# graphic-goose/ferreus_rbf_rs

Measured on AMD Instinct MI355X. Metric: BBFMM matvecs/s, higher is better.
Workload: dtype f64; 1 GPU; 10000000 uniform 3D points, LinearRbf, order 7, 1 rhs, adaptive sparse tree, ACA eps=1e-7, set_weights + evaluate at the sources; points=10000000, kernel=LinearRbf, order=7, nrhs=1, parallelism=single GPU

## Files before the change

ferreus_rbf_rs_amd/_lib.py:

```python
from __future__ import annotations

import ctypes
import os

HERE = os.path.dirname(os.path.abspath(__file__))
LIB_PATH = os.environ.get("FERREUS_BBFMM_HIP_LIB") or os.path.join(HERE, "libferreus_bbfmm_hip.so")

OK, POINT_OUTSIDE_TREE, KERNEL_NO_GRADIENTS, BAD_ARGUMENT, DEVICE_ERROR, UNSUPPORTED = range(6)
FLAG_HOST_ONLY = 1
FLAG_M2L_SHARED_BASIS = 2
FLAG_DIRECT_SMALL_W_LEAVES = 4
FLAG_DETERMINISTIC = 8
N_PHASES = 11
PHASE_NAMES = ["gather", "P2M", "M2M", "M2L_stage1", "M2L_stage2", "P2L", "L2L", "P2P", "M2P",
               "L2P", "scatter"]

c_i32, c_i64, c_f64, c_u32 = ctypes.c_int32, ctypes.c_int64, ctypes.c_double, ctypes.c_uint32
c_p = ctypes.c_void_p


class Params(ctypes.Structure):
    _fields_ = [("max_points_per_cell", c_i64), ("compression_type", c_i32),
                ("epsilon", c_f64), ("eval_chunk_size", c_i64)]

# ... 56 lines not shown
    "bbfmm_isosurface_cluster_tables": (ctypes.c_int, [c_p, c_p, c_p]),
    "bbfmm_isosurface_curvature_tables": (ctypes.c_int, [c_p, c_p, c_p]),
    "bbfmm_isosurface_curvature_weight": (ctypes.c_int, [c_p, c_p, c_i32, c_p, c_p, c_p, c_p]),
    "bbfmm_isosurface_curvature_stats": (ctypes.c_int, [c_p, c_i32, c_p]),
    "bbfmm_isosurface_count": (c_i32, [c_p]),
    "bbfmm_isosurface_size": (ctypes.c_int, [c_p, c_i32, c_p, c_p]),
    "bbfmm_isosurface_copy": (ctypes.c_int, [c_p, c_i32, c_p, c_p]),
    "bbfmm_isosurface_error": (ctypes.c_char_p, [c_p]),
    "bbfmm_isosurface_destroy": (None, [c_p]),
    "bbfmm_prepare_target_subset": (ctypes.c_int, [c_p, c_p, c_i64]),
    "bbfmm_fast_matrix_vector_product": (ctypes.c_int, [c_p, c_p, c_i64, c_i64, c_p, c_i64, c_p,
                                                        c_i64, c_f64, c_p]),
    "bbfmm_matvec_device": (ctypes.c_int, [c_p, c_p, c_i64, c_i32, c_p, c_i64, c_i32]),
    "bbfmm_target_subset_create": (ctypes.c_int, [c_p, c_p, c_i64, c_p]),
    "bbfmm_matvec_subset_device": (ctypes.c_int, [c_p, c_i32, c_p, c_p, c_i32]),
    "bbfmm_stream": (c_p, [c_p]),
    "bbfmm_set_partition": (ctypes.c_int, [c_p, c_i32, c_i32]),
    "bbfmm_partition_row_count": (c_i64, [c_p]),
    "bbfmm_partition_rows": (ctypes.c_int, [c_p, c_p]),
    "bbfmm_partition_coarse_count": (c_i64, [c_p]),
    "bbfmm_matvec_partition_upward": (ctypes.c_int, [c_p, c_p, c_i64, c_i32, c_p, c_p]),
    "bbfmm_matvec_partition_finish": (ctypes.c_int, [c_p, c_p, c_p, c_i64, c_i32, c_p]),
    "bbfmm_partition_world": (c_i32, [c_p]),
    "bbfmm_partition_rank": (c_i32, [c_p]),
    "bbfmm_partition_bounds": (ctypes.c_int, [c_p, c_i32, c_p]),
    "bbfmm_matvec_partition_finish_sorted": (ctypes.c_int, [c_p, c_p, c_p, c_i64, c_p]),
    "bbfmm_partition_scatter": (ctypes.c_int, [c_p, c_p, c_i32, c_i32, c_i64, c_i32, c_p, c_i64]),
    "bbfmm_debug_partition_upward_counts": (ctypes.c_int, [c_p, c_p, c_p, c_p]),
    "bbfmm_debug_host_copy_rates": (ctypes.c_int, [c_i64, c_p]),
    "bbfmm_get_tree_stats": (ctypes.c_int, [c_p, c_p]),
    "bbfmm_tree_built_on_device": (ctypes.c_int, [c_p]),
    "bbfmm_last_evaluate_at_sources": (ctypes.c_int, [c_p]),
    "bbfmm_debug_targets_are_sources": (ctypes.c_int, [c_p, c_p, c_i64, c_i64]),
    "bbfmm_debug_rows_of_sources": (ctypes.c_int, [c_p, c_p, c_i64, c_i64, c_p]),
    "bbfmm_get_cells": (ctypes.c_int, [c_p, c_p, c_p]),
    "bbfmm_get_leaf_sources": (ctypes.c_int, [c_p, c_p, c_p]),
    "bbfmm_get_list": (ctypes.c_int, [c_p, ctypes.c_char, c_p, c_p, c_p]),
    "bbfmm_get_m2l_ranks": (ctypes.c_int, [c_p, c_p, c_p]),
    "bbfmm_get_m2l_operator": (ctypes.c_int, [c_p, c_i32, c_i32, c_p]),
    "bbfmm_get_m2l_factors": (ctypes.c_int, [c_p, c_i32, c_i32, c_p, c_p]),
    "bbfmm_get_permutation_tables": (ctypes.c_int, [c_p, c_p, c_p, c_p, c_p, c_p]),
    "bbfmm_points_to_leaves": (ctypes.c_int, [c_p, c_p, c_i64, c_i64, c_p, c_p]),
    "bbfmm_set_profiling": (ctypes.c_int, [c_p, c_i32]),
    "bbfmm_get_phase_ms": (ctypes.c_int, [c_p, c_p, c_p]),
    "bbfmm_reset_phase_ms": (ctypes.c_int, [c_p]),
    "bbfmm_mfma_f64_selftest": (ctypes.c_int, [c_p, c_p, c_p]),
    "bbfmm_fp64_valu_selftest": (ctypes.c_int, [c_p, c_p]),
    "bbfmm_debug_kernel_values": (ctypes.c_int, [c_i32, c_i32, ctypes.c_double, ctypes.c_double, c_p, c_i64, c_p, c_p, c_p]),
    "bbfmm_debug_math": (ctypes.c_int, [c_i32, c_i32, c_p, c_i64, c_p, c_p]),
    "bbfmm_debug_dense_m2m": (ctypes.c_int, [c_p, c_i32, c_p]),
    "bbfmm_debug_apply_m2l_tables_host": (ctypes.c_int, [c_p, c_p, c_p]),
    "bbfmm_debug_m2l_variants": (ctypes.c_int, [c_p, c_p, c_p]),
    "bbfmm_debug_m2l_pairs": (ctypes.c_int, [c_p, c_p, c_i64, c_p, c_p]),
    "bbfmm_debug_m2l_pairs_stage2": (ctypes.c_int, [c_p, c_p, c_i64, c_p, c_p]),
    "bbfmm_debug_m2l_s2_last_ksplit": (ctypes.c_int, [c_p, c_p]),
    "bbfmm_debug_get_coefficients": (ctypes.c_int, [c_p, ctypes.c_char, c_i32, c_p]),
    "bbfmm_debug_morton_encode": (ctypes.c_uint64, [c_i32, c_p, ctypes.c_uint64]),
    "bbfmm_debug_morton_decode": (None, [c_i32, ctypes.c_uint64, c_p, c_p]),
    "bbfmm_debug_morton_neighbours": (c_i32, [c_i32, ctypes.c_uint64, c_p]),
    "bbfmm_debug_direction_vectors": (c_i32, [c_i32, c_p]),
    "bbfmm_debug_reference_vectors": (ctypes.c_int, [c_p, c_p, c_p]),
    "bbfmm_givens_rotation": (None, [c_f64, c_f64, c_p, c_p, c_p]),
    "bbfmm_fgmres": (ctypes.c_int, [c_i64, c_p, c_p, c_p, c_p, c_p, c_p, c_i32, c_i32, c_i32, c_f64,
                                    c_p, c_p, c_p, c_p, c_p]),
    "bbfmm_schwarz_ddm_solver": (ctypes.c_int, [c_i64, c_p, c_p, c_p, c_p, c_p, c_i32, c_i32, c_f64,
                                                c_p, c_p, c_p, c_p, c_p]),
    "bbfmm_rbf_system_apply": (ctypes.c_int, [c_p, c_p, c_p, c_i64]),
    "bbfmm_ddm_params_defaults": (None, [c_p]),
    "bbfmm_ddm_params_for_points": (None, [c_i64, c_p]),
    "bbfmm_ddm_build": (ctypes.c_int, [c_p, c_i64, c_i32, c_i64, c_p, c_p]),
    "bbfmm_ddm_destroy": (None, [c_p]),
    "bbfmm_ddm_num_levels": (c_i32, [c_p]),
    "bbfmm_ddm_level_size": (c_i64, [c_p, c_i32]),
    "bbfmm_ddm_level_points": (ctypes.c_int, [c_p, c_i32, c_p]),
    "bbfmm_ddm_num_domains": (c_i64, [c_p, c_i32]),
    "bbfmm_ddm_domain_size": (c_i64, [c_p, c_i32, c_i64]),
    "bbfmm_ddm_domain": (ctypes.c_int, [c_p, c_i32, c_i64, c_p, c_p, c_p]),
    "bbfmm_schwarz_create": (ctypes.c_int, [c_p, c_p, c_i64, c_i32, c_i64, c_p, c_p, c_p]),
    "bbfmm_schwarz_create_sharded": (ctypes.c_int, [c_p, c_p, c_i64, c_i32, c_i64, c_p, c_p, c_i32, c_i32, c_p, c_i64, c_p, c_p, c_p]),
    "bbfmm_schwarz_factor_bytes": (c_i64, [c_p]),
    "bbfmm_schwarz_domains_owned": (c_i64, [c_p, c_i32, ctypes.POINTER(c_i64), ctypes.POINTER(c_i64)]),
    "bbfmm_schwarz_destroy": (None, [c_p]),
    "bbfmm_schwarz_basis_size": (c_i64, [c_p]),
    "bbfmm_schwarz_num_levels": (c_i32, [c_p]),
    "bbfmm_schwarz_monomial_matrix": (c_p, [c_p]),
    "bbfmm_debug_evaluate_monomials": (ctypes.c_int, [c_p, c_i64, c_i32, c_i64, c_i32, c_p, c_p, c_p]),
    "bbfmm_schwarz_apply": (ctypes.c_int, [c_p, c_p, c_p, c_i64]),
    "bbfmm_schwarz_level_size": (c_i64, [c_p, c_i32]),
    "bbfmm_schwarz_level_points": (ctypes.c_int, [c_p, c_i32, c_p]),
    "bbfmm_schwarz_debug_level_solve": (ctypes.c_int, [c_p, c_i32, c_p, c_p, c_i64, c_i32]),
    "bbfmm_ddm_debug_level_create": (ctypes.c_int, [c_p, c_i64, c_i32, c_i64, c_i64, c_p, c_p, c_p, c_p, c_i32, c_i32, c_p]),
    "bbfmm_ddm_debug_level_destroy": (None, [c_p]),
    "bbfmm_ddm_debug_level_info": (ctypes.c_int, [c_p, c_p]),
    "bbfmm_ddm_debug_level_layout": (ctypes.c_int, [c_p, c_p, c_p, c_p, c_p, c_p]),
    "bbfmm_ddm_debug_level_assembled": (ctypes.c_int, [c_p, c_p]),
    "bbfmm_ddm_debug_level_factor": (ctypes.c_int, [c_p, c_p]),
    "bbfmm_ddm_debug_level_solve": (ctypes.c_int, [c_p, c_p, c_p, c_i64, c_i32]),
}


class Interpolant(ctypes.Structure):
    _fields_ = [("kernel_type", c_i32), ("polynomial_degree", c_i32), ("nugget", c_f64), ("base_range", c_f64),
                ("total_sill", c_f64), ("flags", c_u32)]


FLAG_GLOBAL_SCALING = 1
# ... 49 lines not shown
```

ferreus_rbf_rs_amd/csrc/capi.cpp:

```cpp
#include <cmath>
#include <cstddef>
#include <cstring>
#include <new>
#include <string>
#include <vector>

#include <algorithm>
#include <chrono>
#include <cstdlib>
#include <memory>

#include "device_group.hpp"
#include "ferreus_bbfmm_hip.h"
#include "fmm_tree.hpp"
#include "isosurface.hpp"
#include "isosurface_curvature.hpp"
#include "isosurface_intersect.hpp"
#include "morton.hpp"

struct bbfmm_handle {
    bbfmm::FmmTree tree;
    std::unique_ptr<bbfmm::DeviceGroup> group;
    std::string err;
};
// ... 1221 lines not shown

int bbfmm_debug_apply_m2l_tables_host(const bbfmm_handle *h, const double *M, double *L) {
    if (!h || !M || !L) return BBFMM_BAD_ARGUMENT;
    return h->tree.debug_apply_m2l_tables_host(M, L);
}

uint64_t bbfmm_debug_morton_encode(int32_t d, const uint64_t *anchor, uint64_t level) {
    if (d < 1 || d > 3 || !anchor) return 0;
    return bbfmm::encode_morton_point(anchor, level, d);
}
void bbfmm_debug_morton_decode(int32_t d, uint64_t key, uint64_t *anchor_out, uint64_t *level_out) {
    if (d < 1 || d > 3 || !anchor_out || !level_out) return;
    bbfmm::decode_key(key, d, anchor_out, level_out);
}
int32_t bbfmm_debug_morton_neighbours(int32_t d, uint64_t key, uint64_t *keys_out) {
    if (d < 1 || d > 3 || !keys_out) return -1;
    return bbfmm::get_neighbours(key, d, keys_out);
}
int32_t bbfmm_debug_direction_vectors(int32_t d, int32_t *out) {
    if (d < 1 || d > 3 || !out) return -1;
    const int(*dirs)[3];
    const int n = bbfmm::direction_vectors(d, &dirs);
    for (int i = 0; i < n; ++i)
        for (int a = 0; a < d; ++a) out[i * d + a] = dirs[i][a];
    return n;
}
int bbfmm_debug_reference_vectors(const bbfmm_handle *h, int32_t *out, int32_t *n_ref_out) {
    if (!h) return BBFMM_BAD_ARGUMENT;
    const bbfmm::Operators &ops = h->tree.ops();
    if (n_ref_out) *n_ref_out = ops.n_ref;
    if (out) std::copy(ops.ref_vecs.begin(), ops.ref_vecs.end(), out);
    return BBFMM_OK;
}

int bbfmm_debug_m2l_variants(const bbfmm_handle *h, int64_t *n_variants, int64_t *n_cells) {
    if (!h) return BBFMM_BAD_ARGUMENT;
    int64_t nv = 0, nc = 0;
    h->tree.m2l_variant_stats(&nv, &nc);
    if (n_variants) *n_variants = nv;
    if (n_cells) *n_cells = nc;
    return BBFMM_OK;
}

int bbfmm_debug_m2l_pairs(const bbfmm_handle *h, int32_t *out, int64_t cap, int64_t *n_out, int32_t *pairs_on) {
    if (!h || !n_out) return BBFMM_BAD_ARGUMENT;
    std::vector<int32_t> v;
    h->tree.debug_m2l_pairs(&v);
    *n_out = static_cast<int64_t>(v.size());
    if (pairs_on) *pairs_on = h->tree.m2l_pairs() ? 1 : 0;
    if (out) std::copy(v.begin(), v.begin() + std::min<int64_t>(cap, *n_out), out);
    return BBFMM_OK;
}

int bbfmm_debug_m2l_pairs_stage2(const bbfmm_handle *h, int32_t *out, int64_t cap, int64_t *n_out, int32_t *pairs_on) {
    if (!h || !n_out) return BBFMM_BAD_ARGUMENT;
    std::vector<int32_t> v;
    h->tree.debug_m2l_pairs_stage2(&v);
    *n_out = static_cast<int64_t>(v.size());
    if (pairs_on) *pairs_on = h->tree.m2l_pairs_stage2() ? 1 : 0;
    if (out) std::copy(v.begin(), v.begin() + std::min<int64_t>(cap, *n_out), out);
    return BBFMM_OK;
}

int bbfmm_debug_m2l_s2_last_ksplit(const bbfmm_handle *h, int32_t *ksplit) {
    if (!h || !ksplit) return BBFMM_BAD_ARGUMENT;
    *ksplit = h->tree.debug_m2l_s2_last_ksplit();
    return BBFMM_OK;
}

int bbfmm_debug_get_coefficients(bbfmm_handle *h, char which, int32_t k, double *out) {
    GUARD(h) return h->tree.debug_get_coefficients(which, k, out);
    END_GUARD(h)
}

}

#include "ddm.hpp"
struct bbfmm_ddm {
    bbfmm::DdmTree tree;
};
extern "C" {
void bbfmm_ddm_params_defaults(bbfmm_ddm_params *out) {
    if (!out) return;
    const bbfmm::DdmParams p;
    out->leaf_threshold = p.leaf_threshold;
    out->overlap_quota = p.overlap_quota;
    out->coarse_ratio = p.coarse_ratio;
    out->coarse_threshold = p.coarse_threshold;
}

void bbfmm_ddm_params_for_points(int64_t n, bbfmm_ddm_params *out) {
    if (!out) return;
    bbfmm_ddm_params_defaults(out);
    out->coarse_threshold = std::max<int64_t>(out->coarse_threshold, n / 470 + 1);
}
int bbfmm_ddm_build(const double *points, int64_t n, int32_t d, int64_t ld, const bbfmm_ddm_params *params,
                    bbfmm_ddm **out) {
    if (!out) return BBFMM_BAD_ARGUMENT;
    *out = nullptr;
    bbfmm::DdmParams p;
    if (params) {
        p.leaf_threshold = params->leaf_threshold;
        p.overlap_quota = params->overlap_quota;
        p.coarse_ratio = params->coarse_ratio;
        p.coarse_threshold = params->coarse_threshold;
    }
// ... 53 lines not shown
```

ferreus_rbf_rs_amd/csrc/device.hpp:

```cpp
#pragma once
#include <hip/hip_runtime.h>

#include <cstdint>

#include "kernels.hpp"

namespace bbfmm {

constexpr int kMaxOrder = 16;
constexpr int kM2lTile = 128;
constexpr int kM2lS1Block = 176;
constexpr int kM2lS1BlockPairs = 160;
constexpr int kM2lSlotWindow = 128;
constexpr int kM2lBlkTwoDst = 1 << 30;

struct DevCheb {
    int p, d, n, n_pad;
    double polyn[kMaxOrder * kMaxOrder];
    double nodes[kMaxOrder];
    double xfer[2 * kMaxOrder * kMaxOrder];
};

struct ChebRef {
    const DevCheb *dev;
    int p, d, n, n_pad;
};

struct M2lClass {
    const double *vt_all;
    const int32_t *row_dst;
    const int32_t *row_dst2;
    const int32_t *blk_t0;
    int32_t n_rows;
    int32_t r_pad16;
    int32_t n_t;
    const double *u_all;
    int32_t k_pad;
    int32_t kp;
    const int32_t *cells;
    int32_t n_cells;
    const int32_t *cslot;
    const int64_t *cbase;
};

struct M2lTileDesc {
    int32_t level_class;
    int32_t first;
    int32_t count;
    int32_t q_first;
    int32_t q_count;
    int32_t pad;
};

void launch_gather_weights(const double *w, int64_t ldw, int K, const int32_t *order, int64_t N,
                           double *w_sorted, hipStream_t s);
void launch_gather_weights_subset(const double *w, int64_t ldw, int K, const int32_t *order, const int32_t *pos, int64_t n_pos,
                                  int64_t N, double *w_sorted, hipStream_t s);
constexpr int kMaxScatterParts = 64;
struct ScatterParts {
    int n;
    int64_t bound[kMaxScatterParts + 1];
};
void launch_scatter_parts(const double *all, const ScatterParts &parts, int64_t m_max, int K, const int32_t *order, double *out,
                          int64_t ldo, hipStream_t s);
void launch_sum_slots(const double *slots, int n_slots, int64_t len, double *out, hipStream_t s);
void launch_scatter_output(const double *out_sorted, int64_t n, int K, const int32_t *perm,
                           double *out, int64_t ldo, int accumulate, hipStream_t s);
void launch_gather_rows(const double *src, int64_t ld_src, int ncols, const int32_t *idx, int64_t n,
                        double *dst, int64_t ld_dst, hipStream_t s);

void launch_p2m(const ChebRef &ch, const double *const *src_xyz, const double *w_sorted, int64_t N,
                int K, int64_t C, const int32_t *leaf_cells, int n_leaves, const int32_t *pt_begin,
                const int32_t *pt_end, const double *centers, const double *lengths, double *M,
                hipStream_t s);
int launch_m2m(const ChebRef &ch, int K, int64_t C, const int32_t *parents, int n_parents,
               const int64_t *child_ptr, const int32_t *child_idx, const int32_t *octant, double *M,
               hipStream_t s);
int launch_l2l(const ChebRef &ch, int K, int64_t C, const int32_t *cells, int n_cells,
               const int32_t *parent, const int32_t *octant, const uint8_t *active, double *L,
               hipStream_t s);

void launch_m2l_stage1(const M2lClass *classes, const M2lTileDesc *tiles, const int32_t *tile_idx, int n_tiles,
                       int n_pad, int max_slot_t, int K, int64_t C, const double *M, double *cbuf,
                       int64_t cbuf_len, hipStream_t s, bool own_blocks = false, int max_blocks = 8, int ne16 = 0);
void launch_m2l_parity(const double *M, int n_pad, double *Mp, int n_par, int ne16, int n_e, int n_o, int p, int64_t rows,
                       hipStream_t s);
void launch_m2l_stage2(const M2lClass *classes, const M2lTileDesc *tiles, const int32_t *tile_idx, int n_tiles,
                       int n_pad, int K, int64_t C, const double *cbuf, int64_t cbuf_len,
                       const uint16_t *qlist, double *L, hipStream_t s, bool allow_ksplit = true);
struct M2lS2PairsPlan {
    int ga, gb, ce, co;
    int ne16() const { return 16 * ga * ce; }
    int n_par() const { return 16 * (ga * ce + gb * co); }
};
M2lS2PairsPlan m2l_s2_pairs_plan(int groups_even, int groups_odd);
bool launch_m2l_stage2_pairs(const M2lClass *classes, const M2lTileDesc *tiles, const int32_t *tile_idx, int n_tiles,
                             const M2lS2PairsPlan &plan, int K, int64_t C, const double *cbuf, int64_t cbuf_len,
                             const uint16_t *qlist, double *Lp, hipStream_t s, bool allow_ksplit = true, int *ksplit_out = nullptr);
void launch_m2l_unparity(const double *Lp, int n_par, int ne16, double *L, int n, int n_pad, int n_e, int n_o, int p, int64_t rows,
                         hipStream_t s);
void launch_m2l_zero_segments(const int32_t *segs, int64_t n_segs, int K, double *cbuf, int64_t cbuf_len, hipStream_t s);
void launch_m2l_basis(const M2lClass *classes, const M2lTileDesc *tiles, int n_tiles, int in_ld, int out_ld, int K,
                      int64_t C, const double *in, double *out, hipStream_t s);
void launch_small_gemm(bool trans_a, int M, int N, int Kd, const double *A, int64_t lda, const double *B, int64_t ldb,
                       double *Cm, int64_t ldc, hipStream_t s);

struct M2lAssembleTv {
    int32_t perm;
    int32_t rank;
    int32_t row;
    int64_t vt_off;
    int64_t u_off;
};
struct M2lAssembleClass {
    const M2lAssembleTv *src, *tgt;
    int32_t n_src, n_tgt, r_pad16, k_pad, max_rank;
    int32_t n_e, n_o, ne16, n_par, p;
    int32_t u_npar, u_ne16, u_rows, u_ne, u_no;
};
void launch_m2l_assemble(const M2lAssembleClass &c, int n, int n_pad, bool compressed, const double *ops,
                         const int32_t *invperm, double *vt_all, double *u_all, hipStream_t s);

struct DirectJobs {
    int n_jobs;
    const int32_t *job_cell;
    const int32_t *tgt_begin, *tgt_end;
    const int64_t *run_ptr;
    const int32_t *runs;
};
void launch_p2p(const KernelSpec &ks, int d, const DirectJobs &jobs, const double *const *tgt_xyz,
                int64_t n_tgt, const double *const *src_xyz, const double *w_sorted, int64_t N, int K,
                double *out_sorted, double *grad_sorted, hipStream_t s);
constexpr int kSymMaxRhs = 4;
void launch_p2p_sym(const KernelSpec &ks, int n_jobs, const int32_t *tgt_begin, const int32_t *tgt_end,
                    const int64_t *run_range, int n_leaf_jobs, const int32_t *l_tgt_begin, const int32_t *l_tgt_end,
                    const int64_t *l_run_range, int n_wave_jobs, const int32_t *w_tgt_begin, const int32_t *w_tgt_end,
                    const int64_t *w_run_range, const int32_t *runs3, int32_t tgt_off, const double *const *src_xyz,
                    const double *w_sorted, int64_t ldw, int K, double *out_sorted, int64_t ldo, hipStream_t s);
int p2p_sym_rows_per_job();
int p2p_sym3_rows_per_job();
int p2p_sym_wave_rows();
int64_t p2p_sym_wave_min_jobs();
int wx_sym_rows_per_job();
int wx_sym3_rows_per_job();
void launch_wx_sym(const KernelSpec &ks, const ChebRef &ch, int n_jobs, const int32_t *tgt_begin, const int32_t *tgt_end,
                   const int64_t *w_range, int n_leaf_jobs, const int32_t *l_tgt_begin, const int32_t *l_tgt_end,
                   const int64_t *l_w_range, const int32_t *w_cells, const double *centers, const double *lengths,
                   const double *const *src_xyz, const double *w_sorted, int64_t ldw, int K, const double *M, double *L,
                   int64_t ld_ml, double *out_sorted, int64_t ldo, int out_off, int out_n, hipStream_t s);
void launch_m2p(const KernelSpec &ks, const ChebRef &ch, int n_jobs, const int32_t *tgt_begin,
                const int32_t *tgt_end, const int64_t *w_begin, const int64_t *w_end,
                const int32_t *w_cells,
                const double *centers, const double *lengths, const double *const *tgt_xyz,
                int64_t n_tgt, int K, int64_t C, const double *M, double *out_sorted,
                double *grad_sorted, hipStream_t s);
void launch_p2l(const KernelSpec &ks, const ChebRef &ch, int n_jobs, const int32_t *cells,
                const int64_t *run_ptr, const int32_t *runs, const double *centers,
                const double *lengths, const double *const *src_xyz, const double *w_sorted,
                int64_t N, int K, int64_t C, double *L, hipStream_t s);
void launch_l2p(const ChebRef &ch, int n_jobs, const int32_t *leaf_cells, const int32_t *tgt_begin,
                const int32_t *tgt_end, const double *centers, const double *lengths,
                const double *const *tgt_xyz, int64_t n_tgt, int K, int64_t C, const double *L,
                double *out_sorted, double *grad_sorted, hipStream_t s);

bool l2p_order_supported(int p, int d);

int mfma_f64_selftest(double *tflops, int *layout_errors, double *info);
int valu_f64_selftest(double *tflops, double *mhz);
int debug_kernel_values_device(const KernelSpec &ks, const double *r2, int64_t n, double *value, double *value_g, double *factor);
int debug_math_device(int which, const double *x, int64_t n, double *out, double *out2);

// ... 2 lines not shown
```

ferreus_rbf_rs_amd/csrc/device_m2l.hip:

```cpp
#include "device_common.hpp"

#include <cmath>

namespace bbfmm {

typedef __attribute__((address_space(3))) void *lptr_t;

__device__ inline unsigned lds_offset(const double *p) {
    return static_cast<unsigned>(reinterpret_cast<uintptr_t>((lptr_t)p));
}
__device__ inline unsigned uniform_u32(unsigned v) { return __builtin_amdgcn_readfirstlane(v); }
__device__ inline const double *uniform_ptr(const double *p) {
    const uintptr_t v = reinterpret_cast<uintptr_t>(p);
    const unsigned lo = __builtin_amdgcn_readfirstlane(static_cast<unsigned>(v));
    const unsigned hi = __builtin_amdgcn_readfirstlane(static_cast<unsigned>(v >> 32));
    return reinterpret_cast<const double *>((static_cast<uintptr_t>(hi) << 32) | lo);
}
__device__ inline void dma16(const double *g, unsigned lds_wave_byte_offset) {
    asm volatile("s_mov_b32 m0, %1\n\ts_nop 0\n\tglobal_load_lds_dwordx4 %0, off" ::"v"(g),
                 "s"(uniform_u32(lds_wave_byte_offset))
                 : "memory");
}
__device__ inline void dma4(const int32_t *g, unsigned lds_wave_byte_offset) {
    asm volatile("s_mov_b32 m0, %1\n\ts_nop 0\n\tglobal_load_lds_dword %0, off" ::"v"(g),
                 "s"(uniform_u32(lds_wave_byte_offset))
                 : "memory");
}
__device__ inline void wait_dma_and_barrier() {
    asm volatile("s_waitcnt vmcnt(0)" ::: "memory");
    __syncthreads();
}
template <int N> __device__ inline void wait_dma_keep_stores_and_barrier() {
    asm volatile("s_waitcnt vmcnt(%0)" ::"n"(N < 63 ? N : 63) : "memory");
    __syncthreads();
}
template <int N> __device__ inline double add_row_ror(double v) {
    const int lo = __double2loint(v), hi = __double2hiint(v);
    const int rlo = __builtin_amdgcn_update_dpp(0, lo, 0x120 + N, 0xf, 0xf, false);
    const int rhi = __builtin_amdgcn_update_dpp(0, hi, 0x120 + N, 0xf, 0xf, false);
    return v + __hiloint2double(rhi, rlo);
}

__device__ inline void dma16s(const double *sbase, unsigned voff_bytes, unsigned lds_wave_byte_offset) {
    asm volatile("s_mov_b32 m0, %2\n\ts_nop 0\n\tglobal_load_lds_dwordx4 %0, %1" ::"v"(voff_bytes),
                 "s"(uniform_ptr(sbase)), "s"(uniform_u32(lds_wave_byte_offset))
                 : "memory");
}

template <int NG16, int STAGE, int MINW, bool PAIRS = false>
__global__ __launch_bounds__(512, MINW) void m2l_gemm_k4(const M2lClass *__restrict__ classes,
                                                  const M2lTileDesc *__restrict__ tiles, int n_pad, int g16_0,
                                                  int64_t C, const double *__restrict__ in, int64_t in_len,
                                                  double *__restrict__ out, int64_t out_len,
                                                  const uint16_t *__restrict__ qlist, int slot_t,
                                                  const int32_t *__restrict__ tile_idx) {
    extern __shared__ double lds[];
    const M2lTileDesc tile = tiles[blockIdx.x];
    const M2lClass cls = classes[tile.level_class];
    const int kr = blockIdx.y;
    const int tid = threadIdx.x, wave = tid >> 6, lane = tid & 63;
    constexpr int BLK = PAIRS ? kM2lS1BlockPairs : kM2lS1Block;
    const int n_zb = STAGE == 1 ? cls.r_pad16 / BLK : 1;
    const bool own_blocks = STAGE == 1 && tile.pad == 2;
    const int zb0 = STAGE == 1 ? (own_blocks ? tile.q_first : (int)((int64_t)n_zb * blockIdx.z / gridDim.z)) : 0;
    const int zb1 = STAGE == 1 ? (own_blocks ? tile.q_first + tile.q_count : (int)((int64_t)n_zb * (blockIdx.z + 1) / gridDim.z)) : 1;
    const int ld = STAGE == 1 ? cls.r_pad16 : n_pad;
    const int ksplit = STAGE == 2 && slot_t > 1 ? slot_t : 1;
    const int zcols = STAGE == 2 ? (int)gridDim.z / ksplit : 1;
    const int zk = STAGE == 2 ? (int)blockIdx.z / zcols : 0, zc = STAGE == 2 ? (int)blockIdx.z - zk * zcols : (int)blockIdx.z;
    const int q_lo = STAGE == 2 ? tile.q_count * zk / ksplit : 0;
    const int nq = STAGE == 1 ? n_pad / 16 : STAGE == 2 ? tile.q_count * (zk + 1) / ksplit - q_lo : (int)(in_len / 16);
    const uint16_t *ql = qlist + tile.q_first + q_lo;
    const int nq_e = PAIRS ? (int)(in_len / 16) : 0;
    if (zb0 >= zb1) return;
    const int g16 = g16_0 + (STAGE >= 2 ? zc * NG16 : 0);
    const double *opbase = (STAGE == 1 ? cls.vt_all : cls.u_all) + 16 * g16;

    constexpr int OP_CHUNKS = 2 * NG16;
    constexpr int NCH = (OP_CHUNKS + 7) / 8;
    constexpr int OP_DOUBLES = OP_CHUNKS * 128;
    constexpr int BUF = OP_DOUBLES + 2048;

    constexpr int NP = NG16 / 2, NS = NG16 & 1;
    unsigned voff[NCH];
#pragma unroll
    for (int i = 0; i < NCH; ++i) {
        const int c = wave + 8 * i;
        if (c < 4 * NP) {
            const int e = c / NP, pr = c - e * NP, k = lane >> 4, p = lane & 15;
            voff[i] = (unsigned)(((4 * k + e) * ld + 32 * pr + 2 * p) * 8);
        } else {
            const int e = 2 * (c - 4 * NP) + (lane >> 5), r = lane & 31, k = r >> 3, pair = r & 7;
            voff[i] = (unsigned)(((4 * k + e) * ld + 32 * NP + 2 * pair) * 8);
        }
    }
    auto cell_p = [&](int pos) {
        const int q = pos < tile.count ? pos : 0;
        return tile.pad ? tile_idx[tile.first + q] : tile.first + q;
    };
    const double *cptr[2];
#pragma unroll
    for (int h = 0; h < 2; ++h) {
        const int tg = 2 * h + (lane >> 5), eh = (lane >> 4) & 1, k = (lane >> 2) & 3, j = lane & 3;
        const int pos = wave * 16 + 4 * tg + j;
        const int p = cell_p(pos);
        const int64_t base = STAGE == 2 ? (int64_t)kr * in_len + cls.cbase[p]
                                        : ((int64_t)kr * C + cls.cells[p]) * (STAGE == 1 ? (int64_t)n_pad : in_len);
        cptr[h] = in + base + 4 * k + 2 * eh;
    }
    const unsigned lds0 = lds_offset(lds);
    const int64_t qstride = (int64_t)16 * ld;
    auto stage = [&](int sidx, int buf) {
        const int zb = zb0 + sidx / nq, qi = sidx - (sidx / nq) * nq;
        const int q = STAGE == 2 ? (int)ql[qi] : qi;
#pragma unroll
        for (int i = 0; i < NCH; ++i)
            if (wave + 8 * i < OP_CHUNKS)
                dma16s(opbase + (int64_t)zb * BLK + q * qstride, voff[i],
                       lds0 + (unsigned)(buf * BUF + (wave + 8 * i) * 128) * 8u);
#pragma unroll
        for (int h = 0; h < 2; ++h)
            dma16(cptr[h] + 16 * q, lds0 + (unsigned)(buf * BUF + OP_DOUBLES + (2 * wave + h) * 128) * 8u);
    };

    double acc[4][NG16];
    double acc_e[4][PAIRS ? NG16 : 1];
#pragma unroll
    for (int tg = 0; tg < 4; ++tg)
#pragma unroll
        for (int g = 0; g < NG16; ++g) {
            acc[tg][g] = 0.0;
            if constexpr (PAIRS) acc_e[tg][g] = 0.0;
        }

    const int bk = lane >> 4, bj = lane & 3;
    const bool wave_live = wave * 16 < tile.count;
    const int n_steps = (zb1 - zb0) * nq;
    const int di = lane >> 4, db = (lane >> 2) & 3, dj = lane & 3;
    constexpr int AUX = PAIRS ? 384 : 192;
    const int32_t *aux = reinterpret_cast<const int32_t *>(lds + 2 * BUF);
    int32_t *ptab = reinterpret_cast<int32_t *>(lds + 2 * BUF) + 2 * AUX;
    const int32_t *slds = aux + 2 * AUX + 128 + wave * 16 * slot_t;
    if (STAGE == 1 && lane < 16) ptab[wave * 16 + lane] = cell_p(wave * 16 + lane);
    const unsigned aux0 = lds0 + (unsigned)(2 * BUF) * 8u;
    auto stage_cols = [&](int zb_, int par) {
        if (STAGE == 1 && 64 * wave <= 16 * NG16) {
            const int e = 64 * wave + lane;
            const int32_t *src = e < 16 * NG16 ? cls.row_dst + zb_ * BLK + 16 * g16 + e : cls.blk_t0 + zb_;
            dma4(src, aux0 + (unsigned)(par * AUX + 64 * wave) * 4u);
        } else if (PAIRS && 64 * wave < 192 + 16 * NG16) {
            const int e = 64 * wave + lane - 192;
            const int32_t *src = e < 16 * NG16 ? cls.row_dst2 + zb_ * BLK + 16 * g16 + e : cls.blk_t0 + zb_;
            dma4(src, aux0 + (unsigned)(par * AUX + 64 * wave) * 4u);
        }
    };
    const int slot_sh = 31 - __builtin_clz(slot_t | 1);
    auto stage_slots = [&](int par) {
        const int t0 = __builtin_amdgcn_readfirstlane(aux[par * AUX + 16 * NG16]) & (kM2lBlkTwoDst - 1);
        const unsigned dst0 = aux0 + (unsigned)(2 * AUX + 128 + wave * 16 * slot_t) * 4u;
        for (int i = 0; i < slot_t / 4; ++i) {
            const int e = i * 64 + lane, cl = e >> slot_sh, tl = e & (slot_t - 1);
            const int32_t *src = cls.cslot + (int64_t)ptab[wave * 16 + cl] * cls.n_t + min(t0 + tl, cls.n_t - 1);
            dma4(src, dst0 + (unsigned)i * 256u);
        }
    };
    if (n_steps > 0) {
        stage(0, 0);
// ... 184 lines not shown
                                int n_pad, int n_colblocks, int K, int64_t C, const double *in, int64_t in_len,
                                double *out, int64_t out_len, const uint16_t *qlist, int slot_t,
                                const int32_t *tile_idx, hipStream_t s) {
    int done = 0;
    const int pref = m2l_chunk_pref<STAGE>();
    while (done < total_groups) {
        const int left = total_groups - done;
        int take;
#define M2L_GO(NG, MW)                                                                                              \
    {                                                                                                               \
        take = NG;                                                                                                  \
        m2l_gemm_launch<NG, STAGE, MW>(classes, tiles, n_tiles, n_pad, done,                                        \
                                       STAGE >= 2 ? 1 : n_colblocks, K, C, in, in_len,                            \
                                       out, out_len, qlist, slot_t, tile_idx, s);                                   \
    }
        if (STAGE >= 2 && !(n_colblocks == 1 && left >= 16)) {
            int best_ng = 2, best_z = 1;
            for (int ng : {11, 8, 7, 6, 4, 2})
                for (int zc = 1; zc <= (n_colblocks == 1 ? 1 : ng == 11 ? 2 : 3); ++zc)
                    if (ng * zc <= left && ((left - ng * zc) % 2 == 0 || left - ng * zc == 7) &&
                        (ng * zc > best_ng * best_z || (ng * zc == best_ng * best_z && ng > best_ng))) {
                        best_ng = ng;
                        best_z = zc;
                    }
            take = best_ng * best_z;
#define M2L_ZGO(NG, MW)                                                                                             \
    m2l_gemm_launch<NG, STAGE, MW>(classes, tiles, n_tiles, n_pad, done, best_z, K, C, in, in_len, out, out_len,    \
                                   qlist, slot_t, tile_idx, s);
            if constexpr (STAGE >= 2) {
                switch (best_ng) {
                case 11: M2L_ZGO(11, 1) break;
                case 8: M2L_ZGO(8, 4) break;
                case 7: M2L_ZGO(7, 2) break;
                case 6: M2L_ZGO(6, 4) break;
                case 4: M2L_ZGO(4, 4) break;
                default: M2L_ZGO(2, 4) break;
                }
            }
#undef M2L_ZGO
        } else if (pref == 22 && left >= 22) M2L_GO(22, 1)
        else if (pref == 22 && left >= 16) M2L_GO(16, 1)
        else if (pref == 11 && left >= 11) M2L_GO(11, 1)
        else if (left >= 8) M2L_GO(8, 4)
        else if (left >= 6) M2L_GO(6, 4)
        else if (left >= 4) M2L_GO(4, 4)
        else M2L_GO(2, 4)
#undef M2L_GO
        done += take;
    }
}

void launch_m2l_stage1(const M2lClass *classes, const M2lTileDesc *tiles, const int32_t *tile_idx, int n_tiles,
                       int n_pad, int max_slot_t, int K, int64_t C, const double *M, double *cbuf, int64_t cbuf_len,
                       hipStream_t s, bool own_blocks, int max_blocks, int ne16) {
    if (n_tiles == 0) return;
    int slot_t = 16;
    while (slot_t < max_slot_t) slot_t *= 2;
    const int n_cu = device_cu_count();
    const int zmax = n_tiles * 8 < n_cu ? std::max(8, std::min(max_blocks, 32)) : 8;
    int zsplit = 1;
    double best = 1e300;
    for (int z = 1; z <= zmax; ++z) {
        const double rounds = std::ceil(static_cast<double>(n_tiles) * z / n_cu);
        const double cost = rounds / z * (1.0 + 0.005 * z);
        if (cost < best - 1e-12) {
            best = cost;
            zsplit = z;
        }
    }
    const int n_colblocks = own_blocks ? 1 : zsplit;
    if (ne16 > 0) {
        m2l_gemm_launch<kM2lS1BlockPairs / 16, 1, 1, true>(classes, tiles, n_tiles, n_pad, 0, n_colblocks, K, C, M, ne16, cbuf, cbuf_len,
                                                      nullptr, slot_t, tile_idx, s);
        return;
    }
    m2l_dispatch_chunks<1>(kM2lS1Block / 16, classes, tiles, n_tiles, n_pad, n_colblocks, K, C, M, 0, cbuf, cbuf_len, nullptr,
                           slot_t, tile_idx, s);
}

static int m2l_s2_ksplit(int64_t wgs, bool allow_ksplit) {
    static const int ks_env = [] {
        const int v = env_int("BBFMM_M2L_S2_KSPLIT", 0);
        return v >= 1 && v <= 32 ? v : 0;
    }();
    if (!allow_ksplit) return 1;
    if (ks_env > 0) return ks_env;
    const int n_cu = device_cu_count();
    int ksplit = 1;
    if (wgs * 2 <= static_cast<int64_t>(kM2lS2KsplitFill) * n_cu) {
        double best = 1e300;
        for (int ks = 1; ks <= 16; ++ks) {
            const double cost = std::ceil(static_cast<double>(wgs * ks) / n_cu) * (0.05 + 1.0 / ks);
            if (cost < best - 1e-12) {
                best = cost;
                ksplit = ks;
            }
        }
    }
    return ksplit;
}

void launch_m2l_stage2(const M2lClass *classes, const M2lTileDesc *tiles, const int32_t *tile_idx, int n_tiles,
                       int n_pad, int K, int64_t C, const double *cbuf, int64_t cbuf_len, const uint16_t *qlist,
                       double *L, hipStream_t s, bool allow_ksplit) {
    if (n_tiles == 0) return;
    static const int z = env_int("BBFMM_M2L_S2_ZSPLIT", 2) == 1 ? 1 : 2;
    const int ksplit = m2l_s2_ksplit(static_cast<int64_t>(n_tiles) * z * K, allow_ksplit);
    m2l_dispatch_chunks<2>(n_pad / 16, classes, tiles, n_tiles, n_pad, z, K, C, cbuf, cbuf_len, L, 0, qlist, ksplit > 1 ? ksplit : 0, tile_idx, s);
}

template <int NG16>
__device__ __forceinline__ void m2l_s2_pairs_body(const M2lClass &cls, const M2lTileDesc &tile, int n_par, int g16, bool odd,
                                                  int zk, int ksplit, int64_t C, const double *__restrict__ in, int64_t in_len,
                                                  double *__restrict__ out, const uint16_t *__restrict__ qlist,
                                                  const int32_t *__restrict__ tile_idx, double *lds) {
    const int kr = blockIdx.y;
    const int tid = threadIdx.x, wave = tid >> 6, lane = tid & 63;
    const int ld = n_par;
    const int q_lo = tile.q_count * zk / ksplit;
    const int nq = tile.q_count * (zk + 1) / ksplit - q_lo;
    const uint16_t *ql = qlist + tile.q_first + q_lo;
    const int kp = cls.kp, kp16 = kp >> 4;
    const double *opbase = cls.u_all + 16 * g16;

    constexpr int OP_CHUNKS = 2 * NG16;
// ... 189 lines not shown
}

__global__ __launch_bounds__(256) void m2l_unparity_kernel(const double *__restrict__ Lp, int n_par, int ne16, double *__restrict__ L,
                                                           int n, int n_pad, int n_e, int n_o, int p, int p1, int64_t rows) {
    const int64_t row = static_cast<int64_t>(blockIdx.x) * 4 + (threadIdx.x >> 6);
    if (row >= rows) return;
    const double *src = Lp + row * n_par;
    double *dst = L + row * n_pad;
    for (int j = threadIdx.x & 63; j < n_e; j += 64) {
        const double e = src[j];
        if (j < n_o) {
            const double o = src[ne16 + j];
            dst[j] = e + o;
            dst[j + (p - 1 - 2 * (j / p1)) * p1] = e - o;
        } else {
            dst[j] = e;
        }
    }
    for (int j = n + (threadIdx.x & 63); j < n_pad; j += 64) dst[j] = 0.0;
}

void launch_m2l_unparity(const double *Lp, int n_par, int ne16, double *L, int n, int n_pad, int n_e, int n_o, int p, int64_t rows,
                         hipStream_t s) {
    if (rows <= 0) return;
    const int p1 = n_e / ((p + 1) / 2);
    hipLaunchKernelGGL(m2l_unparity_kernel, dim3(static_cast<unsigned>((rows + 3) / 4)), dim3(256), 0, s, Lp, n_par, ne16, L, n, n_pad, n_e,
                       n_o, p, p1, rows);
}

__global__ __launch_bounds__(256) void m2l_parity_kernel(const double *__restrict__ M, int n_pad, double *__restrict__ Mp, int n_par,
                                                         int ne16, int n_e, int n_o, int p, int p1, int64_t rows) {
    const int64_t row = static_cast<int64_t>(blockIdx.x) * 4 + (threadIdx.x >> 6);
    if (row >= rows) return;
    const double *src = M + row * n_pad;
    double *dst = Mp + row * n_par;
    for (int j = threadIdx.x & 63; j < n_e; j += 64) {
        const double v = src[j];
        if (j < n_o) {
            const double w = src[j + (p - 1 - 2 * (j / p1)) * p1];
            dst[j] = v + w;
            dst[ne16 + j] = v - w;
        } else {
            dst[j] = v;
        }
    }
}

void launch_m2l_parity(const double *M, int n_pad, double *Mp, int n_par, int ne16, int n_e, int n_o, int p, int64_t rows,
                       hipStream_t s) {
    if (rows <= 0) return;
    const int p1 = n_e / ((p + 1) / 2);
    hipLaunchKernelGGL(m2l_parity_kernel, dim3(static_cast<unsigned>((rows + 3) / 4)), dim3(256), 0, s, M, n_pad, Mp, n_par, ne16, n_e,
                       n_o, p, p1, rows);
}

__global__ __launch_bounds__(256) void m2l_zero_segments_kernel(const int32_t *__restrict__ segs, int64_t n_segs,
                                                                double *__restrict__ cbuf, int64_t cbuf_len) {
    const int64_t sg = (static_cast<int64_t>(blockIdx.x) * 256 + threadIdx.x) >> 4;
    const int l = threadIdx.x & 15;
    if (sg >= n_segs) return;
    const int2 e = reinterpret_cast<const int2 *>(segs)[sg];
    double2 *dst = reinterpret_cast<double2 *>(cbuf + static_cast<int64_t>(blockIdx.y) * cbuf_len) + e.x;
    for (int i = l; i < e.y; i += 16) dst[i] = make_double2(0.0, 0.0);
}

void launch_m2l_zero_segments(const int32_t *segs, int64_t n_segs, int K, double *cbuf, int64_t cbuf_len, hipStream_t s) {
    if (n_segs <= 0) return;
    hipLaunchKernelGGL(m2l_zero_segments_kernel, dim3(static_cast<unsigned>((n_segs * 16 + 255) / 256), K), dim3(256), 0, s, segs,
                       n_segs, cbuf, cbuf_len);
}

void launch_m2l_basis(const M2lClass *classes, const M2lTileDesc *tiles, int n_tiles, int in_ld, int out_ld, int K,
                      int64_t C, const double *in, double *out, hipStream_t s) {
    if (n_tiles == 0) return;
    m2l_dispatch_chunks<3>(out_ld / 16, classes, tiles, n_tiles, out_ld, 2, K, C, in, in_ld, out, 0, nullptr, 0, nullptr, s);
}

template <bool TA>
__global__ __launch_bounds__(256) void small_gemm_kernel(int M, int N, int Kd, const double *__restrict__ A, int64_t lda,
                                                         const double *__restrict__ B, int64_t ldb, double *__restrict__ Cm,
                                                         int64_t ldc) {
    __shared__ double sa[16][64 + 1], sb[16][64 + 1];
    const int tx = threadIdx.x & 15, ty = threadIdx.x >> 4;
    const int i0 = blockIdx.y * 64, j0 = blockIdx.x * 64;
    double acc[4][4] = {};
    for (int k0 = 0; k0 < Kd; k0 += 16) {
        for (int e = threadIdx.x; e < 16 * 64; e += 256) {
            const int kk = TA ? e >> 6 : e & 15, ii = TA ? e & 63 : e >> 4;
            const int k = k0 + kk, i = i0 + ii;
            sa[kk][ii] = (k < Kd && i < M) ? (TA ? A[(int64_t)k * lda + i] : A[(int64_t)i * lda + k]) : 0.0;
        }
        for (int e = threadIdx.x; e < 16 * 64; e += 256) {
            const int kk = e >> 6, jj = e & 63;
            const int k = k0 + kk, j = j0 + jj;
            sb[kk][jj] = (k < Kd && j < N) ? B[(int64_t)k * ldb + j] : 0.0;
        }
        __syncthreads();
#pragma unroll
        for (int kk = 0; kk < 16; ++kk) {
            double a[4], b[4];
#pragma unroll
            for (int r = 0; r < 4; ++r) a[r] = sa[kk][ty + 16 * r];
#pragma unroll
            for (int c = 0; c < 4; ++c) b[c] = sb[kk][tx + 16 * c];
#pragma unroll
            for (int r = 0; r < 4; ++r)
// ... 9 lines not shown
            const int i = i0 + ty + 16 * r, j = j0 + tx + 16 * c;
            if (i < M && j < N) Cm[(int64_t)i * ldc + j] = acc[r][c];
        }
}

void launch_small_gemm(bool trans_a, int M, int N, int Kd, const double *A, int64_t lda, const double *B, int64_t ldb,
                       double *Cm, int64_t ldc, hipStream_t s) {
    if (M <= 0 || N <= 0) return;
    const dim3 grid((N + 63) / 64, (M + 63) / 64);
    if (trans_a) hipLaunchKernelGGL(small_gemm_kernel<true>, grid, dim3(256), 0, s, M, N, Kd, A, lda, B, ldb, Cm, ldc);
    else hipLaunchKernelGGL(small_gemm_kernel<false>, grid, dim3(256), 0, s, M, N, Kd, A, lda, B, ldb, Cm, ldc);
}

__global__ __launch_bounds__(256) void assemble_vt_kernel(M2lAssembleClass c, int n, int n_pad, int compressed,
                                                          const double *__restrict__ ops, const int32_t *__restrict__ invperm,
                                                          double *__restrict__ vt_all) {
    const int64_t t = static_cast<int64_t>(blockIdx.x) * 256 + threadIdx.x;
    if (t >= static_cast<int64_t>(c.n_src) * n) return;
    const int pos = static_cast<int>(t / n), m = static_cast<int>(t % n);
    const M2lAssembleTv tv = c.src[pos];
    const int im = invperm[static_cast<int64_t>(tv.perm) * n + m];
    double *dst = vt_all + static_cast<int64_t>(m) * c.r_pad16 + tv.row;
    if (compressed) {
        const double *src = ops + tv.vt_off + static_cast<int64_t>(im) * tv.rank;
        for (int kk = 0; kk < tv.rank; ++kk) dst[kk] = src[kk];
    } else {
        dst[im] = 1.0;
    }
}

__global__ __launch_bounds__(256) void assemble_vt_parity_kernel(M2lAssembleClass c, int n, const double *__restrict__ ops,
                                                                 const int32_t *__restrict__ invperm, double *__restrict__ vt_all) {
    const int64_t t = static_cast<int64_t>(blockIdx.x) * 256 + threadIdx.x;
    if (t >= static_cast<int64_t>(c.n_src) * c.n_e) return;
    const int pos = static_cast<int>(t / c.n_e), j = static_cast<int>(t % c.n_e);
    const M2lAssembleTv tv = c.src[pos];
    const int p1 = n / c.p;
    const int rj = j + (c.p - 1 - 2 * (j / p1)) * p1;
    const int32_t *inv = invperm + static_cast<int64_t>(tv.perm) * n;
    const double *s0 = ops + tv.vt_off + static_cast<int64_t>(inv[j]) * tv.rank;
    const double *s1 = ops + tv.vt_off + static_cast<int64_t>(inv[rj]) * tv.rank;
    double *de = vt_all + static_cast<int64_t>(j) * c.r_pad16 + tv.row;
    double *dod = vt_all + static_cast<int64_t>(c.ne16 + j) * c.r_pad16 + tv.row;
    if (j >= c.n_o) {
        for (int kk = 0; kk < tv.rank; ++kk) de[kk] = s0[kk];
    } else {
        for (int kk = 0; kk < tv.rank; ++kk) {
            de[kk] = 0.5 * (s0[kk] + s1[kk]);
            dod[kk] = 0.5 * (s0[kk] - s1[kk]);
        }
    }
}

__global__ __launch_bounds__(256) void assemble_u_kernel(M2lAssembleClass c, int n, int n_pad, const double *__restrict__ ops,
                                                         const int32_t *__restrict__ invperm, double *__restrict__ u_all) {
    const int pos = blockIdx.y;
    const M2lAssembleTv tv = c.tgt[pos];
    const int64_t t = static_cast<int64_t>(blockIdx.x) * 256 + threadIdx.x;
    if (t >= static_cast<int64_t>(tv.rank) * n) return;
    const int kk = static_cast<int>(t / n), i = static_cast<int>(t % n);
    u_all[static_cast<int64_t>(tv.row + kk) * n_pad + i] = ops[tv.u_off + static_cast<int64_t>(kk) * n + invperm[static_cast<int64_t>(tv.perm) * n + i]];
}

__global__ __launch_bounds__(256) void assemble_u_parity_kernel(M2lAssembleClass c, int n, const double *__restrict__ ops,
                                                                const int32_t *__restrict__ invperm, double *__restrict__ u_all) {
    const M2lAssembleTv tv = c.tgt[blockIdx.y];
    const int64_t t = static_cast<int64_t>(blockIdx.x) * 256 + threadIdx.x;
    if (t >= static_cast<int64_t>(tv.rank) * c.u_ne) return;
    const int kk = static_cast<int>(t / c.u_ne), i = static_cast<int>(t % c.u_ne);
    const int p1 = n / c.p;
    const int ri = i + (c.p - 1 - 2 * (i / p1)) * p1;
    const int32_t *inv = invperm + static_cast<int64_t>(tv.perm) * n;
    const double *ucol = ops + tv.u_off + static_cast<int64_t>(kk) * n;
    double *dst = u_all + static_cast<int64_t>(tv.row + kk) * c.u_npar;
    const double a = ucol[inv[i]];
    if (i >= c.u_no) {
        dst[i] = a;
    } else {
        const double b = ucol[inv[ri]];
        dst[i] = 0.5 * (a + b);
        dst[c.u_ne16 + i] = 0.5 * (a - b);
    }
}

void launch_m2l_assemble(const M2lAssembleClass &c, int n, int n_pad, bool compressed, const double *ops,
                         const int32_t *invperm, double *vt_all, double *u_all, hipStream_t s) {
    (void)hipMemsetAsync(vt_all, 0, static_cast<size_t>(c.n_e > 0 ? c.n_par : n_pad) * c.r_pad16 * sizeof(double), s);
    (void)hipMemsetAsync(u_all, 0, (c.u_npar > 0 ? static_cast<size_t>(c.u_rows) * c.u_npar : static_cast<size_t>(c.k_pad) * n_pad) * sizeof(double), s);
    if (c.n_src > 0 && c.n_e > 0)
        hipLaunchKernelGGL(assemble_vt_parity_kernel, dim3(static_cast<unsigned>((static_cast<int64_t>(c.n_src) * c.n_e + 255) / 256)), dim3(256),
                           0, s, c, n, ops, invperm, vt_all);
    else if (c.n_src > 0)
        hipLaunchKernelGGL(assemble_vt_kernel, dim3(static_cast<unsigned>((static_cast<int64_t>(c.n_src) * n + 255) / 256)), dim3(256), 0, s, c, n, n_pad,
                           compressed ? 1 : 0, ops, invperm, vt_all);
    if (c.n_tgt > 0 && c.max_rank > 0 && c.u_npar > 0)
        hipLaunchKernelGGL(assemble_u_parity_kernel, dim3(static_cast<unsigned>((static_cast<int64_t>(c.max_rank) * c.u_ne + 255) / 256), c.n_tgt),
                           dim3(256), 0, s, c, n, ops, invperm, u_all);
    else if (c.n_tgt > 0 && c.max_rank > 0)
        hipLaunchKernelGGL(assemble_u_kernel, dim3(static_cast<unsigned>((static_cast<int64_t>(c.max_rank) * n + 255) / 256), c.n_tgt), dim3(256), 0, s, c,
                           n, n_pad, ops, invperm, u_all);
}

}
```

ferreus_rbf_rs_amd/csrc/fmm_m2l_tables.cpp:

```cpp
#include "fmm_tree_impl.hpp"

namespace bbfmm {

void FmmTree::fill_m2l_operator_arrays(const HostM2lClass &hc, std::vector<double> *vt_all,
                                       std::vector<double> *u_all) const {
    const int n_pad = round_up(ops_.n, 32);
    vt_all->resize(static_cast<size_t>(m2l_pairs_ ? m2l_npar_ : n_pad) * hc.r_pad16);
    u_all->resize(m2l_pairs2_ ? static_cast<size_t>(hc.k_pad - hc.kp) * m2l_s2_plan_.n_par() : static_cast<size_t>(hc.k_pad) * n_pad);
    fill_m2l_operator_arrays(hc, vt_all->data(), u_all->data());
}

void FmmTree::fill_m2l_operator_arrays(const HostM2lClass &hc, double *vt_all, double *u_all) const {
    const int n = ops_.n, n_pad = round_up(n, 32);
    const bool compressed = ops_.compression != kCompressionNone;
    const auto &lops = ops_.m2l[hc.level];
    auto zero = [](double *p, size_t len) {
        parallel_for_chunks(static_cast<int64_t>(len), int64_t(1) << 18, [&](int64_t b, int64_t e) {
            std::memset(p + b, 0, static_cast<size_t>(e - b) * sizeof(double));
        });
    };
    zero(vt_all, static_cast<size_t>(m2l_pairs_ ? m2l_npar_ : n_pad) * hc.r_pad16);
    zero(u_all, m2l_pairs2_ ? static_cast<size_t>(hc.k_pad - hc.kp) * m2l_s2_plan_.n_par() : static_cast<size_t>(hc.k_pad) * n_pad);
    struct RowSrc {
        const M2lOperator *op;
        const int32_t *inv;
        int first_row;
    };
    std::vector<RowSrc> row_src;
    for (size_t pos = 0; pos < hc.src_tv.size(); ++pos) {
        if (m2l_pairs_ && hc.src_pair[pos] == -2) continue;
        const int tv = hc.src_tv[pos];
        const M2lOperator &op = lops[ops_.ref_lookup[tv]];
        row_src.push_back(RowSrc{&op, &ops_.invperm[static_cast<size_t>(ops_.perm_lookup[tv]) * n], hc.src_row0[pos]});
    }
    if (m2l_pairs_) {
        parallel_for(m2l_ne_, 8, [&](int64_t j) {
            const bool centre = j >= m2l_no_;
            const int rj = m2l_rho(static_cast<int>(j));
            double *de = vt_all + static_cast<size_t>(j) * hc.r_pad16;
            double *dod = vt_all + static_cast<size_t>(m2l_ne16_ + j) * hc.r_pad16;
            for (const RowSrc &rs : row_src) {
                const int r = rs.op->rank;
                const double *s0 = &rs.op->vt[static_cast<size_t>(rs.inv[j]) * r], *s1 = &rs.op->vt[static_cast<size_t>(rs.inv[rj]) * r];
                for (int kk = 0; kk < r; ++kk) {
                    if (centre) {
                        de[rs.first_row + kk] = s0[kk];
                    } else {
                        de[rs.first_row + kk] = 0.5 * (s0[kk] + s1[kk]);
                        dod[rs.first_row + kk] = 0.5 * (s0[kk] - s1[kk]);
                    }
                }
            }
        });
    } else {
        parallel_for(n, 8, [&](int64_t m) {
            double *dst = vt_all + static_cast<size_t>(m) * hc.r_pad16;
            for (const RowSrc &rs : row_src) {
                const int r = rs.op->rank;
                const int im = rs.inv[m];
                if (compressed) {
                    const double *src = &rs.op->vt[static_cast<size_t>(im) * r];
                    for (int kk = 0; kk < r; ++kk) dst[rs.first_row + kk] = src[kk];
                } else {
                    dst[rs.first_row + im] = 1.0;
                }
            }
        });
    }
    if (m2l_pairs2_) {
        const int n_par = m2l_s2_plan_.n_par(), ne16 = m2l_s2_plan_.ne16();
        parallel_for(static_cast<int64_t>(hc.tgt_tv.size()), 1, [&](int64_t pos) {
            if (hc.tgt_pair[pos] == -2) return;
            const int tv = hc.tgt_tv[pos];
            const M2lOperator &op = lops[ops_.ref_lookup[tv]];
            const int32_t *inv = &ops_.invperm[static_cast<size_t>(ops_.perm_lookup[tv]) * n];
            const int row0 = hc.tgt_off[pos] - (hc.tgt_pair[pos] >= 0 ? 0 : hc.kp);
            for (int kk = 0; kk < op.rank; ++kk) {
                double *dst = u_all + static_cast<size_t>(row0 + kk) * n_par;
                const double *ucol = &op.u[static_cast<size_t>(kk) * n];
                for (int i = 0; i < m2l_ne_; ++i) {
                    const double a = ucol[inv[i]], b = ucol[inv[m2l_rho(i)]];
                    if (i >= m2l_no_) {
                        dst[i] = a;
                    } else {
                        dst[i] = 0.5 * (a + b);
                        dst[ne16 + i] = 0.5 * (a - b);
                    }
                }
// ... 22 lines not shown
    m2l_variants_.clear();
    m2l_tiles1_h_.clear();
    m2l_tile_idx1_h_.clear();
    m2l_classes_h_.clear();
    m2l_tiles_h_.clear();
    m2l_qlist_h_.clear();
    m2l_batches_.clear();
    m2l_batch_of_class_.clear();
    m2l_group_ops_.clear();
    cbuf_batch_len_ = 0;
    cbuf_total_len_ = 0;
    m2l_flops_k1_ = 0;
    m2l_flops_level_.clear();
    if (t.depth < 2) return BBFMM_OK;
    if (!host_only_) {
        size_t free_b = 0, total_b = 0;
        if (hipMemGetInfo(&free_b, &total_b) == hipSuccess && total_b > 0)
            m2l_budget_bytes_ = std::max<int64_t>(int64_t(4) << 30, static_cast<int64_t>(total_b / 16));
    }
    if (const char *e = std::getenv("BBFMM_M2L_CBUF_MB")) {
        const double mb = std::atof(e);
        if (mb > 0) m2l_budget_bytes_ = static_cast<int64_t>(mb * 1048576.0);
    }

    auto comp = [&](int tv, int a) { return ops_.all_vecs[static_cast<size_t>(tv) * d + a]; };
    {
        const char *e = std::getenv("BBFMM_M2L_S1_PAIRS");
        m2l_pairs_ = !(e && std::atoi(e) == 0) && compressed && !shared_basis_ && d >= 2 && ops_.p >= 2;
        const char *e2 = std::getenv("BBFMM_M2L_S2_PAIRS");
        m2l_pairs2_ = !(e2 && std::atoi(e2) == 0) && compressed && !shared_basis_ && d >= 2 && ops_.p >= 2;
        m2l_partner_.assign(static_cast<size_t>(nvec), -1);
        m2l_s1_block_ = m2l_pairs_ ? kM2lS1BlockPairs : kM2lS1Block;
        const int p1 = n / ops_.p;
        m2l_ne_ = (ops_.p + 1) / 2 * p1;
        m2l_no_ = ops_.p / 2 * p1;
        m2l_ne16_ = round_up(m2l_ne_, 16);
        m2l_npar_ = m2l_ne16_ + round_up(m2l_no_, 16);
        m2l_s2_plan_ = m2l_s2_pairs_plan(m2l_ne16_ / 16, round_up(m2l_no_, 16) / 16);
        for (int tv = 0; tv < nvec && (m2l_pairs_ || m2l_pairs2_); ++tv) {
            if (comp(tv, 0) == 0) continue;
            int rt = -1;
            for (int u = 0; u < nvec && rt < 0; ++u) {
                bool same = comp(u, 0) == -comp(tv, 0);
                for (int a = 1; a < d; ++a) same = same && comp(u, a) == comp(tv, a);
                if (same) rt = u;
            }
            if (rt < 0 || ops_.ref_lookup[rt] != ops_.ref_lookup[tv]) continue;
            const int32_t *it = &ops_.invperm[static_cast<size_t>(ops_.perm_lookup[tv]) * n];
            const int32_t *ir = &ops_.invperm[static_cast<size_t>(ops_.perm_lookup[rt]) * n];
            bool ok = true;
            for (int m = 0; m < n && ok; ++m) ok = ir[m] == it[m2l_rho(m)];
            if (ok) m2l_partner_[static_cast<size_t>(tv)] = rt;
        }
    }
    auto far = [&](int tv) {
        int mx = 0;
        for (int a = 0; a < d; ++a) mx = std::max(mx, std::abs(comp(tv, a)));
        return mx >= 2;
    };
    std::vector<std::vector<int>> tgt_list(ncls), src_list(ncls), tpos_tgt(ncls, std::vector<int>(nvec, -1)),
        tpos_src(ncls, std::vector<int>(nvec, -1));
    for (int o = 0; o < ncls; ++o)
        for (int tv = 0; tv < nvec; ++tv) {
            if (!far(tv)) continue;
            bool okt = true, oks = true;
            for (int a = 0; a < d; ++a) {
                const int oa = (o >> a) & 1, ta = comp(tv, a);
                okt = okt && ta >= oa - 3 && ta <= oa + 2;
                oks = oks && ta >= -2 - oa && ta <= 3 - oa;
            }
            if (okt) {
                tpos_tgt[o][tv] = static_cast<int>(tgt_list[o].size());
                tgt_list[o].push_back(tv);
            }
            if (oks) {
                tpos_src[o][tv] = static_cast<int>(src_list[o].size());
                src_list[o].push_back(tv);
            }
        }
    auto pairs_first = [&](std::vector<int> *list, std::vector<int> *tpos) {
        std::vector<int> ordered, singles;
        std::vector<uint8_t> used(static_cast<size_t>(nvec), 0);
        for (int tv : *list) {
            const int rt = m2l_partner_[static_cast<size_t>(tv)];
            if (used[static_cast<size_t>(tv)]) continue;
            if (rt >= 0 && (*tpos)[rt] >= 0 && m2l_partner_[static_cast<size_t>(rt)] == tv) {
                const int first = comp(tv, 0) > 0 ? tv : rt;
                ordered.push_back(first);
                ordered.push_back(first == tv ? rt : tv);
                used[static_cast<size_t>(tv)] = used[static_cast<size_t>(rt)] = 1;
            } else {
                singles.push_back(tv);
            }
        }
        ordered.insert(ordered.end(), singles.begin(), singles.end());
        *list = ordered;
        for (size_t i = 0; i < ordered.size(); ++i) (*tpos)[ordered[i]] = static_cast<int>(i);
    };
    for (int o = 0; o < ncls; ++o) {
        if (m2l_pairs_) pairs_first(&src_list[o], &tpos_src[o]);
        if (m2l_pairs2_) pairs_first(&tgt_list[o], &tpos_tgt[o]);
    }
    std::vector<std::vector<int32_t>> tgt_pair(ncls);
    for (int o = 0; o < ncls; ++o) {
        const std::vector<int> &tl = tgt_list[o];
        tgt_pair[o].assign(tl.size(), -1);
        for (size_t pos = 0; m2l_pairs2_ && pos + 1 < tl.size(); ++pos)
            if (m2l_partner_[static_cast<size_t>(tl[pos])] == tl[pos + 1] && m2l_partner_[static_cast<size_t>(tl[pos + 1])] == tl[pos]) {
                tgt_pair[o][pos] = static_cast<int32_t>(pos + 1);
                tgt_pair[o][pos + 1] = -2;
                ++pos;
            }
    }
    auto target_class = [&](int o, int tv) {
        int oc = 0;
        for (int a = 0; a < d; ++a) {
            const int v = ((o >> a) & 1) + comp(tv, a);
            oc |= (((v % 2) + 2) % 2) << a;
        }
        return oc;
    };

    std::vector<int32_t> pos_in_class(t.n_cells(), -1);
    int64_t bad_pairs = 0;
    auto slot_layout = [&](int level, std::vector<std::vector<int>> *off_tgt, std::vector<int> *k_pad, std::vector<int> *kp_out = nullptr) {
        const auto &lops = ops_.m2l[level];
        off_tgt->assign(ncls, {});
        k_pad->assign(ncls, 0);
        if (kp_out) kp_out->assign(ncls, 0);
        for (int o = 0; o < ncls; ++o) {
            int lead = 0;
            for (size_t pos = 0; pos < tgt_list[o].size(); ++pos)
                if (tgt_pair[o][pos] >= 0) lead += round_up(lops[ops_.ref_lookup[tgt_list[o][pos]]].rank, 2);
            const int kp = round_up(lead, 16);
            int off = 0, off_s = 2 * kp;
            for (size_t pos = 0; pos < tgt_list[o].size(); ++pos) {
                const int seg = round_up(lops[ops_.ref_lookup[tgt_list[o][pos]]].rank, 2);
                if (tgt_pair[o][pos] >= 0) {
                    (*off_tgt)[o].push_back(off);
                } else if (tgt_pair[o][pos] == -2) {
                    (*off_tgt)[o].push_back(kp + off);
                    off += seg;
                } else {
                    (*off_tgt)[o].push_back(off_s);
                    off_s += seg;
                }
            }
            (*k_pad)[o] = round_up(std::max(off_s, 16), 16);
            if (kp_out) (*kp_out)[o] = kp;
        }
    };
    std::vector<int> level_groups(static_cast<size_t>(t.depth) + 1, 1);
    std::vector<std::vector<int>> batch_of(static_cast<size_t>(t.depth) + 1, std::vector<int>(ncls, -1));
    {
// ... 8 lines not shown
        int64_t cur_len = 0;
        for (int level = 2; level <= t.depth; ++level) {
            int64_t len = 0;
            for (int64_t v : class_len[level]) len += v;
            cbuf_total_len_ += len;
            int G = 1;
            if (len > budget)
                for (G = 2; G < ncls; G *= 2) {
                    int64_t worst = 0;
                    for (int g = 0; g < G; ++g) {
                        int64_t gl = 0;
                        for (int o = g * ncls / G; o < (g + 1) * ncls / G; ++o) gl += class_len[level][o];
                        worst = std::max(worst, gl);
                    }
                    if (worst <= budget) break;
                }
            if (G >= ncls) {
                G = ncls;
                int64_t worst = 0;
                for (int64_t v : class_len[level]) worst = std::max(worst, v);
                if (worst > budget && std::getenv("BBFMM_VERBOSE"))
                    std::fprintf(stderr, "[bbfmm] warning: level %d needs %.1f MB of M2L intermediate per right-hand side even "
                                         "with one batch per target class; the budget of %.1f MB (BBFMM_M2L_CBUF_MB) is exceeded\n",
                                 level, worst * 8.0 / 1048576.0, m2l_budget_bytes_ / 1048576.0);
            }
            level_groups[level] = G;
            if (G == 1 && !m2l_batches_.empty() && m2l_batches_.back().groups == 1 && cur_len + len <= budget) {
                m2l_batches_.back().level_hi = level;
                cur_len += len;
                for (int o = 0; o < ncls; ++o) batch_of[level][o] = static_cast<int>(m2l_batches_.size()) - 1;
                continue;
            }
            for (int g = 0; g < G; ++g) {
                M2lBatch b;
                b.level_lo = b.level_hi = level;
                b.groups = G;
                b.group = g;
                for (int o = g * ncls / G; o < (g + 1) * ncls / G; ++o) batch_of[level][o] = static_cast<int>(m2l_batches_.size());
                m2l_batches_.push_back(b);
            }
            cur_len = len;
        }
    }
    std::vector<std::vector<M2lTileDesc>> tiles1_of_batch(m2l_batches_.size());
    std::vector<int32_t> variant_batch;
    std::vector<std::vector<int32_t>> zero_of_batch(m2l_batches_.size());
    for (int level = 2; level <= t.depth; ++level) {
        const auto &lops = ops_.m2l[level];
        auto rank_of = [&](int tv) { return lops[ops_.ref_lookup[tv]].rank; };
        std::vector<std::vector<int>> off_tgt;
        std::vector<int> k_pad, kp_cls;
        slot_layout(level, &off_tgt, &k_pad, &kp_cls);
        const size_t first_class = m2l_host_.size();
        auto mark_pairs = [&](const std::vector<int> &tvs, std::vector<int32_t> *src_pair, std::vector<int32_t> *row0 = nullptr) {
            src_pair->assign(tvs.size(), -1);
            for (size_t pos = 0; m2l_pairs_ && pos + 1 < tvs.size(); ++pos)
                if (m2l_partner_[static_cast<size_t>(tvs[pos])] == tvs[pos + 1] && m2l_partner_[static_cast<size_t>(tvs[pos + 1])] == tvs[pos]) {
                    (*src_pair)[pos] = static_cast<int32_t>(pos + 1);
                    (*src_pair)[pos + 1] = -2;
                    ++pos;
                }
            if (row0) row0->assign(tvs.size(), 0);
            int rows = 0, blk = -1, blk_first = 0;
            for (size_t pos = 0; pos < tvs.size(); ++pos) {
                if ((*src_pair)[pos] == -2) continue;
                const int r = rank_of(tvs[pos]);
                if (r == 0) continue;
                const int last = (*src_pair)[pos] >= 0 ? static_cast<int>(pos) + 1 : static_cast<int>(pos);
                if (rows / m2l_s1_block_ == blk && last - blk_first + 1 > kM2lSlotWindow) rows = round_up(rows, m2l_s1_block_);
                if (row0) (*row0)[pos] = rows;
                const int b1 = (rows + r - 1) / m2l_s1_block_;
                if (rows / m2l_s1_block_ != blk || b1 != blk) {
                    blk = b1;
                    blk_first = static_cast<int>(pos);
                }
                rows = round_up(rows + r, 2);
            }
            return rows;
        };
        auto stage1_rows = [&](int o, const std::vector<int> &tvs, HostM2lClass *hcp) {
            HostM2lClass &hc = *hcp;
            hc.n_t = static_cast<int>(tvs.size());
            std::vector<int32_t> first_row;
            hc.n_rows = mark_pairs(tvs, &hc.src_pair, &first_row);
            hc.r_pad16 = round_up(std::max(hc.n_rows, 1), m2l_s1_block_);
            hc.row_tpos.assign(hc.r_pad16, -1);
            hc.row_off.assign(hc.r_pad16, 0);
            hc.row_tpos2.assign(hc.r_pad16, -1);
            hc.row_off2.assign(hc.r_pad16, 0);
            hc.src_tv = tvs;
            int row = 0;
            hc.src_row0.assign(tvs.size(), 0);
            hc.src_row1.assign(tvs.size(), 0);
            for (size_t pos = 0; pos < tvs.size(); ++pos) {
                if (hc.src_pair[pos] == -2) {
                    hc.src_row0[pos] = hc.src_row0[pos - 1];
                    hc.src_row1[pos] = hc.src_row1[pos - 1];
                    continue;
                }
                const int tv = tvs[pos];
                const int oc = target_class(o, tv);
                const int base_off = off_tgt[oc][tpos_tgt[oc][tv]];
                int base_off2 = 0;
                if (hc.src_pair[pos] >= 0) {
                    const int tv2 = tvs[pos + 1], oc2 = target_class(o, tv2);
                    base_off2 = off_tgt[oc2][tpos_tgt[oc2][tv2]];
                }
                if (rank_of(tv) > 0) row = first_row[pos];
                hc.src_row0[pos] = row;
                for (int kk = 0; kk < rank_of(tv); ++kk, ++row) {
                    hc.row_tpos[row] = static_cast<int32_t>(pos);
                    hc.row_off[row] = base_off + kk;
                    if (hc.src_pair[pos] >= 0) {
                        hc.row_tpos2[row] = static_cast<int32_t>(pos + 1);
                        hc.row_off2[row] = base_off2 + kk;
                    }
                }
                hc.src_row1[pos] = row;
                row = round_up(row, 2);
            }
            const int n_blk = hc.r_pad16 / m2l_s1_block_;
            m2l_max_blocks_ = std::max(m2l_max_blocks_, n_blk);
            hc.blk_t0.assign(n_blk, 0);
            hc.row_dst.assign(hc.r_pad16, -1);
            hc.row_dst2.assign(hc.r_pad16, -1);
            for (int b = 0; b < n_blk; ++b) {
                int t0 = -1, t1 = -1;
                bool two = false;
                for (int r = b * m2l_s1_block_; r < (b + 1) * m2l_s1_block_; ++r) {
                    if (hc.row_tpos[r] < 0) continue;
                    if (t0 < 0) t0 = hc.row_tpos[r];
                    t1 = std::max(hc.row_tpos[r], hc.row_tpos2[r]);
                    two = two || hc.row_tpos2[r] >= 0;
                }
                if (t0 < 0) continue;
                hc.blk_t0[b] = t0 | (two ? kM2lBlkTwoDst : 0);
                m2l_slot_t_ = std::max(m2l_slot_t_, t1 - t0 + 1);
                for (int r = b * m2l_s1_block_; r < (b + 1) * m2l_s1_block_; ++r) {
// ... 120 lines not shown
            const int64_t n_tiles_cls = (static_cast<int64_t>(hc.cells.size()) + kM2lTile - 1) / kM2lTile;
            std::vector<std::vector<uint16_t>> tile_q(static_cast<size_t>(n_tiles_cls));
            parallel_for(n_tiles_cls, 4, [&](int64_t ti) {
                const int32_t first = static_cast<int32_t>(ti * kM2lTile);
                const int32_t count = std::min<int32_t>(kM2lTile, static_cast<int32_t>(hc.cells.size()) - first);
                std::vector<uint8_t> act(static_cast<size_t>(nq), 0);
                for (int32_t i = 0; i < count; ++i) {
                    const int64_t B = hc.cells[first + i];
                    for (int64_t q = t.v.ptr[B]; q < t.v.ptr[B + 1]; ++q) {
                        const int tv = t.v_tidx[q];
                        const int pos = tpos_tgt[o][tv];
                        if (pos < 0) continue;
                        const int a = off_tgt[o][pos] - (off_tgt[o][pos] >= hc.kp ? hc.kp : 0), b = a + rank_of(tv);
                        for (int sq = a / 16; sq <= (b - 1) / 16; ++sq) act[sq] = 1;
                    }
                }
                for (int sq = 0; sq < nq; ++sq)
                    if (act[sq]) tile_q[static_cast<size_t>(ti)].push_back(static_cast<uint16_t>(sq));
            });
            for (int64_t ti = 0; ti < n_tiles_cls; ++ti) {
                M2lTileDesc td;
                td.level_class = static_cast<int32_t>(first_class + o);
                td.first = static_cast<int32_t>(ti * kM2lTile);
                td.count = std::min<int32_t>(kM2lTile, static_cast<int32_t>(hc.cells.size()) - td.first);
                td.pad = 0;
                td.q_first = static_cast<int32_t>(m2l_qlist_h_.size());
                m2l_qlist_h_.insert(m2l_qlist_h_.end(), tile_q[static_cast<size_t>(ti)].begin(), tile_q[static_cast<size_t>(ti)].end());
                td.q_count = static_cast<int32_t>(m2l_qlist_h_.size()) - td.q_first;
                m2l_tiles_h_.push_back(td);
            }
        }
        const int variant_min_tiles = [] {
            const char *e = std::getenv("BBFMM_M2L_VARIANTS");
            return e ? std::atoi(e) : 4;
        }();
        const int G = level_groups[level];
        const bool variants_on = variant_min_tiles > 0 && G == 1;
        for (int g = 0; g < G && G > 1; ++g) {
            const int o_lo = g * ncls / G, o_hi = (g + 1) * ncls / G;
            for (int o = 0; o < ncls; ++o) {
                const HostM2lClass &hc = m2l_host_[first_class + o];
                const size_t nc = hc.cells.size();
                if (nc == 0) continue;
                const int nt = hc.n_t;
                std::vector<int> tvs, keep;
                for (int ps = 0; ps < nt; ++ps) {
                    const int oc = target_class(o, hc.src_tv[ps]);
                    if (oc >= o_lo && oc < o_hi) {
                        tvs.push_back(hc.src_tv[ps]);
                        keep.push_back(ps);
                    }
                }
                if (tvs.empty()) continue;
                HostM2lClass v;
                v.level = level;
                v.octant = o;
                v.k_pad = 16;
                if (!stage1_rows(o, tvs, &v)) return fail(BBFMM_BAD_ARGUMENT, "M2L slot too long for the packed row table");
                v.cells = hc.cells;
                v.cslot.resize(nc * tvs.size());
                {
                    int32_t *dst = v.cslot.data();
                    const int32_t *src = hc.cslot.data();
                    const size_t nk = keep.size();
                    parallel_for_chunks(static_cast<int64_t>(nc), 4096, [&](int64_t lo, int64_t hi) {
                        for (int64_t k = lo; k < hi; ++k)
                            for (size_t q = 0; q < nk; ++q) dst[static_cast<size_t>(k) * nk + q] = src[static_cast<size_t>(k) * nt + keep[q]];
                    });
                }
                const int bidx = batch_of[level][o_lo];
                for (size_t f = 0; f < nc; f += kM2lTile) {
                    M2lTileDesc td;
                    std::memset(&td, 0, sizeof td);
                    td.level_class = -1 - static_cast<int32_t>(m2l_variants_.size());
                    td.first = static_cast<int32_t>(f);
                    td.count = static_cast<int32_t>(std::min<size_t>(kM2lTile, nc - f));
                    td.pad = 0;
                    tiles1_of_batch[static_cast<size_t>(bidx)].push_back(td);
                }
                if (host_only_) fill_m2l_operator_arrays(v, &v.vt_all, &v.u_all);
                m2l_group_ops_[first_class + o].push_back(static_cast<int32_t>(m2l_variants_.size()));
                variant_batch.push_back(bidx);
                m2l_variants_.push_back(std::move(v));
            }
        }
        for (int o = 0; o < ncls && G == 1; ++o) {
            const HostM2lClass &hc = m2l_host_[first_class + o];
            const size_t nc = hc.cells.size();
            if (nc == 0) continue;
            const int nt = hc.n_t;
            std::vector<M2lTileDesc> &tiles1_out = tiles1_of_batch[static_cast<size_t>(batch_of[level][o])];
            std::vector<uint64_t> sig(nc);
            parallel_for(static_cast<int64_t>(nc), 256, [&](int64_t i) {
                uint64_t h = 1469598103934665603ull;
                const int32_t *row = &hc.cslot[static_cast<size_t>(i) * nt];
                uint64_t word = 0;
                for (int ps = 0; ps < nt; ++ps) {
                    word = (word << 1) | (row[ps] >= 0 ? 1u : 0u);
                    if ((ps & 63) == 63 || ps == nt - 1) {
                        h = (h ^ word) * 1099511628211ull;
                        word = 0;
                    }
                }
                sig[static_cast<size_t>(i)] = h;
            });
            auto same_pattern = [&](size_t a, size_t b) {
                if (sig[a] != sig[b]) return false;
                const int32_t *ra = &hc.cslot[a * nt], *rb = &hc.cslot[b * nt];
                for (int ps = 0; ps < nt; ++ps)
                    if ((ra[ps] >= 0) != (rb[ps] >= 0)) return false;
                return true;
            };
            std::vector<int32_t> rest;
            size_t i = 0;
            while (i < nc) {
                size_t j = i + 1;
                while (j < nc && same_pattern(i, j)) ++j;
                size_t full = 0;
                if (variants_on && j - i >= static_cast<size_t>(variant_min_tiles) * kM2lTile) {
                    std::vector<int> tvs;
                    for (int ps = 0; ps < nt; ++ps)
                        if (hc.cslot[i * nt + ps] >= 0) tvs.push_back(hc.src_tv[ps]);
                    std::vector<int32_t> marks;
                    const int present_rows = mark_pairs(tvs, &marks);
                    auto n_pairs = [](const std::vector<int32_t> &m) { return std::count_if(m.begin(), m.end(), [](int32_t v) { return v >= 0; }); };
                    if (!tvs.empty() && (round_up(present_rows, m2l_s1_block_) < hc.r_pad16 || n_pairs(marks) < n_pairs(hc.src_pair))) {
                        full = (j - i) / kM2lTile * kM2lTile;
                        HostM2lClass v;
                        v.level = level;
                        v.octant = o;
                        v.k_pad = 16;
                        if (!stage1_rows(o, tvs, &v)) return fail(BBFMM_BAD_ARGUMENT, "M2L slot too long for the packed row table");
                        v.cells.assign(hc.cells.begin() + static_cast<std::ptrdiff_t>(i), hc.cells.begin() + static_cast<std::ptrdiff_t>(i + full));
                        v.cslot.resize(full * tvs.size());
                        size_t pv = 0;
                        std::vector<int> keep;
                        for (int ps = 0; ps < nt; ++ps)
                            if (hc.cslot[i * nt + ps] >= 0) keep.push_back(ps);
                        for (size_t k = 0; k < full; ++k)
                            for (int ps : keep) v.cslot[pv++] = hc.cslot[(i + k) * nt + ps];
                        for (size_t f = 0; f < full; f += kM2lTile) {
                            M2lTileDesc td;
                            std::memset(&td, 0, sizeof td);
                            td.level_class = -1 - static_cast<int32_t>(m2l_variants_.size());
                            td.first = static_cast<int32_t>(f);
                            td.count = kM2lTile;
                            td.pad = 0;
                            tiles1_out.push_back(td);
                        }
                        if (host_only_) fill_m2l_operator_arrays(v, &v.vt_all, &v.u_all);
                        variant_batch.push_back(batch_of[level][o]);
                        m2l_variants_.push_back(std::move(v));
                    }
                }
                for (size_t k = i + full; k < j; ++k) rest.push_back(static_cast<int32_t>(k));
                i = j;
            }
            for (size_t f = 0; f < rest.size(); f += kM2lTile) {
                M2lTileDesc td;
                std::memset(&td, 0, sizeof td);
                td.level_class = static_cast<int32_t>(first_class + o);
                td.first = static_cast<int32_t>(m2l_tile_idx1_h_.size() + f);
                td.count = static_cast<int32_t>(std::min<size_t>(kM2lTile, rest.size() - f));
                td.pad = 1;
                tiles1_out.push_back(td);
            }
            m2l_tile_idx1_h_.insert(m2l_tile_idx1_h_.end(), rest.begin(), rest.end());
        }
    }
    if (bad_pairs > 0)
        return fail(BBFMM_UNSUPPORTED,
                    "V-list pairs outside the admissible transfer-vector set (source points outside the root box?)");
    m2l_batch_of_class_.assign(m2l_host_.size() + m2l_variants_.size(), 0);
    for (size_t lc = 0; lc < m2l_host_.size(); ++lc)
        m2l_batch_of_class_[lc] = batch_of[static_cast<size_t>(m2l_host_[lc].level)][static_cast<size_t>(m2l_host_[lc].octant)];
    for (size_t v = 0; v < m2l_variants_.size(); ++v) m2l_batch_of_class_[m2l_host_.size() + v] = variant_batch[v];
    m2l_tiles2_h_.clear();
    {
        size_t next = 0;
        for (size_t b = 0; b < m2l_batches_.size(); ++b) {
            M2lBatch &mb = m2l_batches_[b];
            mb.t1_first = static_cast<int32_t>(m2l_tiles1_h_.size());
            for (M2lTileDesc td : tiles1_of_batch[b]) {
                if (td.level_class < 0) td.level_class = static_cast<int32_t>(m2l_host_.size()) + (-1 - td.level_class);
                m2l_tiles1_h_.push_back(td);
            }
            mb.t1_count = static_cast<int32_t>(m2l_tiles1_h_.size()) - mb.t1_first;
            std::vector<M2lTileDesc> part;
            while (next < m2l_tiles_h_.size() && m2l_batch_of_class_[static_cast<size_t>(m2l_tiles_h_[next].level_class)] == static_cast<int32_t>(b))
                part.push_back(m2l_tiles_h_[next++]);
            split_tile_tail(&part, n_cu_);
// ... 228 lines not shown
    const int64_t C = tree_.n_cells();
    double flops = 0.0;
    for (size_t lv = 2; lv < n_levels; ++lv) {
        std::memset(&classes[2 * lv], 0, 2 * sizeof(M2lClass));
        if (basis_rank_[lv] == 0 || lv >= level_cells_.size() || level_cells_[lv].empty()) continue;
        const int rank = basis_rank_[lv];
        std::vector<double> wc(static_cast<size_t>(n_pad) * basis_pad_, 0.0), we(static_cast<size_t>(basis_pad_) * n_pad, 0.0);
        for (int j = 0; j < rank; ++j) {
            const double *col = &basis[lv][static_cast<size_t>(j) * n];
            for (int m = 0; m < n; ++m) {
                wc[static_cast<size_t>(m) * basis_pad_ + j] = col[m];
                we[static_cast<size_t>(j) * n_pad + m] = col[m];
            }
        }
        CHK(dupload(&d_basis_c_[lv], wc));
        CHK(dupload(&d_basis_e_[lv], we));
        const int32_t nc = static_cast<int32_t>(level_cells_[lv].size());
        for (int e = 0; e < 2; ++e) {
            M2lClass &c = classes[2 * lv + e];
            c.u_all = e == 0 ? d_basis_c_[lv].p : d_basis_e_[lv].p;
            c.cells = d_level_cells_[lv].p;
            c.n_cells = nc;
        }
        for (int32_t first = 0; first < nc; first += kM2lTile) {
            const int32_t count = std::min<int32_t>(kM2lTile, nc - first);
            tiles_c.push_back(M2lTileDesc{static_cast<int32_t>(2 * lv), first, count, 0, 0, 0});
            tiles_e.push_back(M2lTileDesc{static_cast<int32_t>(2 * lv + 1), first, count, 0, 0, 0});
        }
        const double lf = lv < m2l_flops_level_.size() ? m2l_flops_level_[lv] : 0.0;
        flops += lf * rank / n + 4.0 * n * rank * nc;
    }
    m2l_flops_k1_ = flops;
    n_basis_tiles_ = static_cast<int>(tiles_c.size());
    CHK(dupload(&d_basis_classes_, classes));
    CHK(dupload(&d_basis_tiles_c_, tiles_c));
    CHK(dupload(&d_basis_tiles_e_, tiles_e));
    (void)C;
    if (std::getenv("BBFMM_VERBOSE")) {
        std::fprintf(stderr, "[bbfmm] shared basis: %d coordinates per cell (n = %d), ranks per level:", basis_pad_, n);
        for (size_t lv = 2; lv < n_levels; ++lv) std::fprintf(stderr, " %d", basis_rank_[lv]);
        std::fprintf(stderr, "\n");
    }
    return BBFMM_OK;
}

int FmmTree::debug_apply_m2l_tables_host(const double *M, double *L) const {
    const int n = ops_.n, n_pad = round_up(n, 32);
    std::vector<double> Mp;
    if (m2l_pairs_) {
        Mp.assign(static_cast<size_t>(tree_.n_cells()) * m2l_npar_, 0.0);
        for (int64_t c = 0; c < tree_.n_cells(); ++c) {
            const double *Mv = M + static_cast<size_t>(c) * n;
            double *mp = &Mp[static_cast<size_t>(c) * m2l_npar_];
            for (int j = 0; j < m2l_ne_; ++j) {
                if (j < m2l_no_) {
                    mp[j] = Mv[j] + Mv[m2l_rho(j)];
                    mp[m2l_ne16_ + j] = Mv[j] - Mv[m2l_rho(j)];
                } else {
                    mp[j] = Mv[j];
                }
            }
        }
    }
    std::vector<double> cbuf(static_cast<size_t>(std::max<int64_t>(cbuf_batch_len_, 1)), 0.0);
    std::vector<int32_t> seen(static_cast<size_t>(tree_.n_cells()), 0);
    const bool have_zero_lists = m2l_batches_.size() > 1 && !m2l_zero_h_.empty();
    for (size_t b = 0; b < m2l_batches_.size(); ++b) {
        const M2lBatch &mb = m2l_batches_[b];
        if (have_zero_lists)
            for (int64_t z = m2l_zero_ptr_[b]; z < m2l_zero_ptr_[b + 1]; ++z)
                std::fill(cbuf.begin() + 2 * static_cast<int64_t>(m2l_zero_h_[static_cast<size_t>(2 * z)]),
                          cbuf.begin() + 2 * (static_cast<int64_t>(m2l_zero_h_[static_cast<size_t>(2 * z)]) + m2l_zero_h_[static_cast<size_t>(2 * z + 1)]), 0.0);
        for (int32_t ti = mb.t1_first; ti < mb.t1_first + mb.t1_count; ++ti) {
            const M2lTileDesc &td = m2l_tiles1_h_[static_cast<size_t>(ti)];
            const bool variant = static_cast<size_t>(td.level_class) >= m2l_host_.size();
            const HostM2lClass &hc = variant ? m2l_variants_[static_cast<size_t>(td.level_class) - m2l_host_.size()]
                                             : m2l_host_[static_cast<size_t>(td.level_class)];
            if (hc.vt_all.empty()) return BBFMM_UNSUPPORTED;
            if (m2l_batch_of_class_[static_cast<size_t>(td.level_class)] != static_cast<int32_t>(b)) return BBFMM_BAD_ARGUMENT;
            for (int32_t q = 0; q < td.count; ++q) {
                const size_t pos = static_cast<size_t>(td.pad ? m2l_tile_idx1_h_[static_cast<size_t>(td.first + q)] : td.first + q);
                ++seen[hc.cells[pos]];
                const double *Mv = M + static_cast<size_t>(hc.cells[pos]) * n;
                for (int row = 0; row < hc.n_rows; ++row) {
                    if (hc.row_tpos[row] < 0) continue;
                    const int32_t slot = hc.cslot[pos * hc.n_t + hc.row_tpos[row]];
                    if (m2l_pairs_) {
                        const int32_t slot2 = hc.row_tpos2[row] >= 0 ? hc.cslot[pos * hc.n_t + hc.row_tpos2[row]] : -1;
                        if (slot < 0 && slot2 < 0) continue;
                        const double *mp = &Mp[static_cast<size_t>(hc.cells[pos]) * m2l_npar_];
                        double a = 0.0, bsum = 0.0;
                        for (int j = 0; j < m2l_ne16_; ++j) a += hc.vt_all[static_cast<size_t>(j) * hc.r_pad16 + row] * mp[j];
                        for (int j = m2l_ne16_; j < m2l_npar_; ++j) bsum += hc.vt_all[static_cast<size_t>(j) * hc.r_pad16 + row] * mp[j];
                        if (slot >= 0) cbuf[static_cast<size_t>(slot) * 2 + hc.row_off[row]] = a + bsum;
                        if (slot2 >= 0) cbuf[static_cast<size_t>(slot2) * 2 + hc.row_off2[row]] = a - bsum;
                        continue;
                    }
                    if (slot < 0) continue;
                    double s = 0.0;
                    for (int m = 0; m < n; ++m) s += hc.vt_all[static_cast<size_t>(m) * hc.r_pad16 + row] * Mv[m];
                    cbuf[static_cast<size_t>(slot) * 2 + hc.row_off[row]] = s;
                }
            }
        }
        for (size_t lc = 0; lc < m2l_host_.size(); ++lc) {
            if (m2l_batch_of_class_[lc] != static_cast<int32_t>(b)) continue;
            const HostM2lClass &hc = m2l_host_[lc];
            for (size_t pos = 0; pos < hc.cells.size(); ++pos) {
                double *Lb = L + static_cast<size_t>(hc.cells[pos]) * n;
                const double *cc = &cbuf[static_cast<size_t>(hc.cbase[pos])];
                if (m2l_pairs2_) {
                    const int n_par = m2l_s2_plan_.n_par(), ne16 = m2l_s2_plan_.ne16(), rows = hc.k_pad - hc.kp;
                    std::vector<double> sm(static_cast<size_t>(rows)), df(static_cast<size_t>(rows));
                    for (int r = 0; r < rows; ++r) {
                        sm[static_cast<size_t>(r)] = r < hc.kp ? cc[r] + cc[hc.kp + r] : cc[hc.kp + r];
                        df[static_cast<size_t>(r)] = r < hc.kp ? cc[r] - cc[hc.kp + r] : cc[hc.kp + r];
                    }
                    for (int i = 0; i < m2l_ne_; ++i) {
                        double le = 0.0, lo = 0.0;
                        for (int r = 0; r < rows; ++r) {
                            le += hc.u_all[static_cast<size_t>(r) * n_par + i] * sm[static_cast<size_t>(r)];
                            lo += hc.u_all[static_cast<size_t>(r) * n_par + ne16 + i] * df[static_cast<size_t>(r)];
                        }
                        if (i >= m2l_no_) {
                            Lb[i] += le;
                        } else {
                            Lb[i] += le + lo;
                            Lb[m2l_rho(i)] += le - lo;
                        }
                    }
                    continue;
                }
                for (int i = 0; i < n; ++i) {
                    double s = 0.0;
                    for (int k = 0; k < hc.k_pad; ++k) s += hc.u_all[static_cast<size_t>(k) * n_pad + i] * cc[k];
                    Lb[i] += s;
                }
            }
        }
    }
    for (const HostM2lClass &hc : m2l_host_)
        for (int32_t c : hc.cells) {
            const size_t lc = static_cast<size_t>(&hc - m2l_host_.data());
            const M2lBatch &mb = m2l_batches_[static_cast<size_t>(m2l_batch_of_class_[lc])];
            const int want = mb.groups == 1 || m2l_group_ops_[lc].empty() ? mb.groups : static_cast<int>(m2l_group_ops_[lc].size());
            if (seen[c] != want) return BBFMM_BAD_ARGUMENT;
        }
    return BBFMM_OK;
}

void FmmTree::debug_m2l_pairs(std::vector<int32_t> *out) const {
    out->clear();
    const int d = d_;
    for (size_t i = 0; i < m2l_host_.size() + m2l_variants_.size(); ++i) {
        const HostM2lClass &h = i < m2l_host_.size() ? m2l_host_[i] : m2l_variants_[i - m2l_host_.size()];
        if (h.cells.empty()) continue;
        out->push_back(h.level);
        out->push_back(h.octant);
        out->push_back(i < m2l_host_.size() ? 0 : 1);
        const size_t n_at = out->size();
        out->push_back(0);
        int32_t n_entries = 0;
        for (size_t pos = 0; pos < h.src_tv.size(); ++pos) {
            if (h.src_pair[pos] == -2) continue;
            out->push_back(h.src_pair[pos] >= 0 ? 1 : 0);
            for (int a = 0; a < d; ++a) out->push_back(ops_.all_vecs[static_cast<size_t>(h.src_tv[pos]) * d + a]);
            ++n_entries;
        }
        (*out)[n_at] = n_entries;
    }
}

void FmmTree::debug_m2l_pairs_stage2(std::vector<int32_t> *out) const {
    out->clear();
    const int d = d_;
    for (const HostM2lClass &h : m2l_host_) {
        if (h.cells.empty()) continue;
        out->push_back(h.level);
        out->push_back(h.octant);
        out->push_back(0);
        const size_t n_at = out->size();
        out->push_back(0);
        int32_t n_entries = 0;
        for (size_t pos = 0; pos < h.tgt_tv.size(); ++pos) {
            if (h.tgt_pair[pos] == -2) continue;
            out->push_back(h.tgt_pair[pos] >= 0 ? 1 : 0);
            for (int a = 0; a < d; ++a) out->push_back(ops_.all_vecs[static_cast<size_t>(h.tgt_tv[pos]) * d + a]);
            ++n_entries;
        }
        (*out)[n_at] = n_entries;
    }
}

}
```

ferreus_rbf_rs_amd/csrc/fmm_tree.cpp:

```cpp
#include "fmm_tree_impl.hpp"

namespace bbfmm {

int FmmTree::fail(int code, const std::string &msg) {
    err_ = msg;
    return code;
}
int FmmTree::hip_fail(hipError_t e, const char *what) {
    err_ = std::string("HIP error: ") + hipGetErrorString(e) + " in " + what;
    return BBFMM_DEVICE_ERROR;
}

void FmmTree::arena_begin() {
    arena_active_ = true;
    arena_used_ = 0;
    arena_need_ = 0;
}
int FmmTree::arena_end() {
    arena_active_ = false;
    if (arena_need_ > arena_.n) {
        dfree(&arena_);
        CHK(dalloc(&arena_, arena_need_ + arena_need_ / 4));
    }
    return BBFMM_OK;
// ... 400 lines not shown
    CHK(dupload(&d_u_runs_, u_runs_.idx));
    CHK(dupload(&d_w_ptr_, t.w.ptr));
    CHK(dupload(&d_w_idx_, t.w.idx));
    {
        std::vector<int64_t> job_ptr(x_cells_.size() + 1, 0);
        std::vector<int32_t> job_runs;
        for (size_t j = 0; j < x_cells_.size(); ++j) {
            const int32_t c = x_cells_[j];
            for (int64_t r = x_runs_.ptr[c]; r < x_runs_.ptr[c + 1]; ++r) {
                job_runs.push_back(x_runs_.idx[2 * r]);
                job_runs.push_back(x_runs_.idx[2 * r + 1]);
            }
            job_ptr[j + 1] = static_cast<int64_t>(job_runs.size() / 2);
        }
        CHK(dupload(&d_x_cells_, x_cells_));
        CHK(dupload(&d_x_job_run_ptr_, job_ptr));
        CHK(dupload(&d_x_runs_, job_runs));
    }
    StageTimer ut;
    HIPCHK(hipStreamSynchronize(stream_));
    ut.lap("  upload: tree, run lists");
    m2l_classes_h_.resize(m2l_host_.size() + m2l_variants_.size());
    const bool compressed = ops_.compression != kCompressionNone;
    DevBuf<int32_t> d_invperm;
    CHK(dupload(&d_invperm, ops_.invperm));
    std::vector<DevBuf<double>> d_level_ops(ops_.m2l.size());
    std::vector<std::vector<int64_t>> u_off(ops_.m2l.size()), vt_off(ops_.m2l.size());
    for (size_t lv = 0; lv < ops_.m2l.size(); ++lv) {
        std::vector<double> buf;
        for (const M2lOperator &op : ops_.m2l[lv]) {
            u_off[lv].push_back(static_cast<int64_t>(buf.size()));
            buf.insert(buf.end(), op.u.begin(), op.u.end());
            vt_off[lv].push_back(static_cast<int64_t>(buf.size()));
            buf.insert(buf.end(), op.vt.begin(), op.vt.end());
        }
        if (!buf.empty()) CHK(dupload(&d_level_ops[lv], buf));
    }
    if (shared_basis_) {
        if (!compressed) return fail(BBFMM_BAD_ARGUMENT, "BBFMM_FLAG_M2L_SHARED_BASIS needs compressed M2L operators (ACA or SVD)");
        CHK(build_shared_basis(&d_level_ops));
    }
    const int m2l_len = shared_basis_ ? basis_pad_ : cheb_.n_pad;
    std::vector<DevBuf<double>> natural_tmp;
    std::vector<DevBuf<M2lAssembleTv>> assemble_tmp;
    for (size_t i = 0; i < m2l_host_.size() + m2l_variants_.size(); ++i) {
        HostM2lClass &h = i < m2l_host_.size() ? m2l_host_[i] : m2l_variants_[i - m2l_host_.size()];
        M2lClass &c = m2l_classes_h_[i];
        std::memset(&c, 0, sizeof c);
        c.n_rows = h.n_rows;
        c.r_pad16 = h.r_pad16;
        c.n_t = h.n_t;
        c.k_pad = h.k_pad;
        c.kp = h.kp;
        c.n_cells = static_cast<int32_t>(h.cells.size());
        if (h.cells.empty()) continue;
        DevBuf<double> vt, ua;
        DevBuf<int32_t> rt, rt2, ro, ce, cs;
        DevBuf<int64_t> cb;
        {
            const size_t nvt = static_cast<size_t>(m2l_pairs_ ? m2l_npar_ : cheb_.n_pad) * h.r_pad16, nu = m2l_pairs2_ ? static_cast<size_t>(h.k_pad - h.kp) * m2l_s2_plan_.n_par() : static_cast<size_t>(h.k_pad) * cheb_.n_pad;
            CHK(dalloc(&vt, nvt));
            CHK(dalloc(&ua, nu));
            const auto &lops = ops_.m2l[h.level];
            std::vector<M2lAssembleTv> src_tv, tgt_tv;
            int max_rank = 0;
            for (size_t pos = 0; pos < h.src_tv.size(); ++pos) {
                if (m2l_pairs_ && h.src_pair[pos] == -2) continue;
                const int tv = h.src_tv[pos];
                const int ref = ops_.ref_lookup[tv];
                const int rank = lops[ref].rank;
                src_tv.push_back(M2lAssembleTv{ops_.perm_lookup[tv], rank, h.src_row0[pos], vt_off[h.level][ref], u_off[h.level][ref]});
            }
            for (size_t pos = 0; pos < h.tgt_tv.size(); ++pos) {
                if (m2l_pairs2_ && h.tgt_pair[pos] == -2) continue;
                const int tv = h.tgt_tv[pos];
                const int ref = ops_.ref_lookup[tv];
                const int rank = lops[ref].rank;
                max_rank = std::max(max_rank, rank);
                const int row = m2l_pairs2_ && h.tgt_pair[pos] < 0 ? h.tgt_off[pos] - h.kp : h.tgt_off[pos];
                tgt_tv.push_back(M2lAssembleTv{ops_.perm_lookup[tv], rank, row, vt_off[h.level][ref], u_off[h.level][ref]});
            }
            DevBuf<M2lAssembleTv> d_src, d_tgt;
            CHK(dupload(&d_src, src_tv));
            CHK(dupload(&d_tgt, tgt_tv));
            const M2lAssembleClass ac{d_src.p, d_tgt.p, static_cast<int32_t>(src_tv.size()), static_cast<int32_t>(tgt_tv.size()),
                                      h.r_pad16, h.k_pad, max_rank,
                                      m2l_pairs_ ? m2l_ne_ : 0, m2l_no_, m2l_ne16_, m2l_npar_, ops_.p,
                                      m2l_pairs2_ ? m2l_s2_plan_.n_par() : 0, m2l_s2_plan_.ne16(), h.k_pad - h.kp, m2l_ne_, m2l_no_};
            static const bool host_fill = std::getenv("BBFMM_M2L_ASSEMBLE_HOST") != nullptr;
            if (host_fill) {
                std::vector<double> hv, hu;
                fill_m2l_operator_arrays(h, &hv, &hu);
                HIPCHK(hipMemcpy(vt.p, hv.data(), hv.size() * sizeof(double), hipMemcpyHostToDevice));
                HIPCHK(hipMemcpy(ua.p, hu.data(), hu.size() * sizeof(double), hipMemcpyHostToDevice));
            } else {
                launch_m2l_assemble(ac, ops_.n, cheb_.n_pad, compressed, d_level_ops[h.level].p, d_invperm.p, vt.p, ua.p, stream_);
            }
            assemble_tmp.push_back(d_src);
            assemble_tmp.push_back(d_tgt);
            if (shared_basis_) {
                DevBuf<double> vt2, ua2;
                CHK(dalloc(&vt2, static_cast<size_t>(m2l_len) * h.r_pad16));
                CHK(dalloc(&ua2, static_cast<size_t>(h.k_pad) * m2l_len));
                const double *W = d_basis_c_[static_cast<size_t>(h.level)].p;
                launch_small_gemm(true, m2l_len, h.r_pad16, cheb_.n_pad, W, m2l_len, vt.p, h.r_pad16, vt2.p, h.r_pad16, stream_);
                launch_small_gemm(false, h.k_pad, m2l_len, cheb_.n_pad, ua.p, cheb_.n_pad, W, m2l_len, ua2.p, m2l_len, stream_);
                natural_tmp.push_back(vt);
                natural_tmp.push_back(ua);
                vt = vt2;
                ua = ua2;
            }
        }
        CHK(dupload(&rt, h.row_dst));
        CHK(dupload(&rt2, h.row_dst2));
        CHK(dupload(&ro, h.blk_t0));
        CHK(dupload(&ce, h.cells));
        CHK(dalloc(&cs, h.cslot.size()));
        if (!h.cslot.empty()) HIPCHK(hipMemcpy(cs.p, h.cslot.data(), h.cslot.size() * sizeof(int32_t), hipMemcpyHostToDevice));
        CHK(dupload(&cb, h.cbase));
        c.vt_all = vt.p;
        c.u_all = ua.p;
        c.row_dst = rt.p;
        c.row_dst2 = rt2.p;
        c.blk_t0 = ro.p;
        c.cells = ce.p;
        c.cslot = cs.p;
        c.cbase = cb.p;
        decltype(h.cslot)().swap(h.cslot);
    }
    HIPCHK(hipStreamSynchronize(stream_));
    HIPCHK(hipGetLastError());
    for (auto &b : assemble_tmp) dfree(&b);
    for (auto &b : natural_tmp) dfree(&b);
    for (auto &b : d_level_ops) dfree(&b);
    dfree(&d_invperm);
    ut.lap("  upload: M2L operators, tables");
    CHK(dupload(&d_m2l_classes_, m2l_classes_h_));
    CHK(dupload(&d_m2l_tiles_, m2l_tiles_h_));
    CHK(dupload(&d_m2l_tiles1_, m2l_tiles1_h_));
    CHK(dupload(&d_tile_idx1_, m2l_tile_idx1_h_));
    CHK(dupload(&d_m2l_tiles2_, m2l_tiles2_h_));
// ... 256 lines not shown
                same.store(false, std::memory_order_relaxed);
        });
    }
    return same.load();
}

int FmmTree::upward(int k, const DownwardPlan *dp) {
    const HostTree &t = tree_;
    const int64_t C = t.n_cells();
    const bool part = dp && dp->restrict_upward;
    multipoles_partial_ = part;
    phase_begin();
    if (part) {
        for (int j = 0; j < k && dp->coarse_cells > 0; ++j)
            HIPCHK(hipMemsetAsync(d_M_.p + static_cast<size_t>(j) * C * cheb_.n_pad, 0,
                                  static_cast<size_t>(dp->coarse_cells) * cheb_.n_pad * sizeof(double), stream_));
        launch_p2m(cheb_, src_ptr_, d_w_sorted_.p, t.n_points, k, C, dp->d_up_leaves.p, static_cast<int>(dp->up_leaves_h.size()),
                   d_pt_begin_.p, d_pt_end_.p, d_centers_.p, d_lengths_.p, d_M_.p, stream_);
    } else {
        launch_p2m(cheb_, src_ptr_, d_w_sorted_.p, t.n_points, k, C, d_src_leaves_.p, static_cast<int>(src_leaves_.size()),
                   d_pt_begin_.p, d_pt_end_.p, d_centers_.p, d_lengths_.p, d_M_.p, stream_);
    }
    phase_end(kPhP2M);
    phase_begin();
    for (int level = t.depth - 1; level >= 1; --level) {
        const int rc = part ? launch_m2m(cheb_, k, C, dp->d_up_parents[level].p, static_cast<int>(dp->up_parents_h[level].size()),
                                         dp->d_part_child_ptr.p, dp->d_part_child_idx.p, d_octant_.p, d_M_.p, stream_)
                            : launch_m2m(cheb_, k, C, d_m2m_parents_[level].p, static_cast<int>(m2m_parents_[level].size()),
                                         d_child_ptr_.p, d_child_idx_.p, d_octant_.p, d_M_.p, stream_);
        if (rc != 0) return hip_fail(static_cast<hipError_t>(rc), "M2M: dynamic LDS attribute");
    }
    phase_end(kPhM2M);
    HIPCHK(hipGetLastError());
    return BBFMM_OK;
}

int FmmTree::downward(int k, const DownwardPlan *dp, const TargetSet *wx) {
    CHK(downward_m2l(k, dp));
    return downward_tail(k, dp, wx);
}

int FmmTree::downward_m2l(int k, const DownwardPlan *dp) {
    const HostTree &t = tree_;
    const int64_t C = t.n_cells();
    have_locals_ = false;
    const bool s2_pairs = m2l_pairs2_ && !m2l_batches_.empty();
    const int lp_len = m2l_s2_plan_.n_par();
    if (!s2_pairs) HIPCHK(hipMemsetAsync(d_L_.p, 0, static_cast<size_t>(k) * C * cheb_.n_pad * sizeof(double), stream_));
    const int m2l_len = shared_basis_ ? basis_pad_ : cheb_.n_pad;
    const double *m_in = shared_basis_ ? d_Mc_.p : m2l_pairs_ ? d_Mp_.p : d_M_.p;
    const int s1_len = m2l_pairs_ ? m2l_npar_ : m2l_len, s1_ne16 = m2l_pairs_ ? m2l_ne16_ : 0;
    if (m2l_pairs_ && !m2l_batches_.empty()) {
        phase_begin();
        launch_m2l_parity(d_M_.p, cheb_.n_pad, d_Mp_.p, m2l_npar_, m2l_ne16_, m2l_ne_, m2l_no_, ops_.p, static_cast<int64_t>(k) * C, stream_);
        phase_end(kPhM2L1);
    }
    double *l_out = shared_basis_ ? d_Lc_.p : s2_pairs ? d_Lp_.p : d_L_.p;
    if (shared_basis_) {
        phase_begin();
        launch_m2l_basis(d_basis_classes_.p, d_basis_tiles_c_.p, n_basis_tiles_, cheb_.n_pad, basis_pad_, k, C, d_M_.p, d_Mc_.p, stream_);
        HIPCHK(hipMemsetAsync(d_Lc_.p, 0, static_cast<size_t>(k) * C * basis_pad_ * sizeof(double), stream_));
        phase_end(kPhM2L1);
    }
    const int nb = static_cast<int>(m2l_batches_.size());
    for (int k0 = 0; k0 < k; k0 += m2l_rhs_chunk_) {
        const int kb = std::min(m2l_rhs_chunk_, k - k0);
        const double *m_chunk = m_in + static_cast<size_t>(k0) * C * s1_len;
        double *l_chunk = s2_pairs ? d_Lp_.p : l_out + static_cast<size_t>(k0) * C * m2l_len;
        if (s2_pairs) HIPCHK(hipMemsetAsync(d_Lp_.p, 0, static_cast<size_t>(kb) * C * lp_len * sizeof(double), stream_));
        for (int b = 0; b < nb; ++b) {
            const M2lBatch &mb = m2l_batches_[static_cast<size_t>(b)];
            const int t1_first = dp ? dp->batch_t1[4 * b] : mb.t1_first, t1_count = dp ? dp->batch_t1[4 * b + 1] : mb.t1_count;
            const int t2_first = dp ? dp->batch_t2[2 * b] : mb.t2_first, t2_count = dp ? dp->batch_t2[2 * b + 1] : mb.t2_count;
            if (t2_count == 0) continue;
            phase_begin();
            if (nb > 1)
                launch_m2l_zero_segments(d_m2l_zero_.p + 2 * m2l_zero_ptr_[static_cast<size_t>(b)],
                                         m2l_zero_ptr_[static_cast<size_t>(b) + 1] - m2l_zero_ptr_[static_cast<size_t>(b)], kb, d_cbuf_.p,
                                         cbuf_batch_len_, stream_);
            if (dp) {
                launch_m2l_stage1(d_m2l_classes_.p, dp->d_tiles1.p + t1_first, dp->d_tile_idx.p, t1_count, s1_len, m2l_slot_t_, kb,
                                  C, m_chunk, d_cbuf_.p, cbuf_batch_len_, stream_, false, m2l_max_blocks_, s1_ne16);
                launch_m2l_stage1(d_m2l_classes_.p, dp->d_tiles1.p + dp->batch_t1[4 * b + 2], dp->d_tile_idx.p, dp->batch_t1[4 * b + 3],
                                  s1_len, m2l_slot_t_, kb, C, m_chunk, d_cbuf_.p, cbuf_batch_len_, stream_, true, m2l_max_blocks_, s1_ne16);
            } else
                launch_m2l_stage1(d_m2l_classes_.p, d_m2l_tiles1_.p + t1_first, d_tile_idx1_.p, t1_count, s1_len, m2l_slot_t_, kb, C,
                                  m_chunk, d_cbuf_.p, cbuf_batch_len_, stream_, false, m2l_max_blocks_, s1_ne16);
            phase_end(kPhM2L1);
            phase_begin();
            if (s2_pairs) {
                if (!launch_m2l_stage2_pairs(d_m2l_classes_.p, dp ? dp->d_tiles2.p + t2_first : d_m2l_tiles2_.p + t2_first,
                                             dp ? dp->d_tile_idx.p : nullptr, t2_count, m2l_s2_plan_, kb, C, d_cbuf_.p, cbuf_batch_len_,
                                             dp ? dp->d_qlist.p : d_m2l_qlist_.p, l_chunk, stream_, !deterministic_, &m2l_s2_last_ksplit_))
                    return fail(BBFMM_DEVICE_ERROR, "internal: no stage-2 kernel instance for the parity-basis column plan");
            } else if (dp)
                launch_m2l_stage2(d_m2l_classes_.p, dp->d_tiles2.p + t2_first, dp->d_tile_idx.p, t2_count, m2l_len, kb, C, d_cbuf_.p,
                                  cbuf_batch_len_, dp->d_qlist.p, l_chunk, stream_, !deterministic_);
            else
                launch_m2l_stage2(d_m2l_classes_.p, d_m2l_tiles2_.p + t2_first, nullptr, t2_count, m2l_len, kb, C, d_cbuf_.p,
                                  cbuf_batch_len_, d_m2l_qlist_.p, l_chunk, stream_, !deterministic_);
            phase_end(kPhM2L2);
        }
        if (s2_pairs) {
            phase_begin();
            launch_m2l_unparity(d_Lp_.p, lp_len, m2l_s2_plan_.ne16(), d_L_.p + static_cast<size_t>(k0) * C * cheb_.n_pad, ops_.n, cheb_.n_pad,
                                m2l_ne_, m2l_no_, ops_.p, static_cast<int64_t>(kb) * C, stream_);
            phase_end(kPhM2L2);
        }
    }
    if (shared_basis_) {
        phase_begin();
        launch_m2l_basis(d_basis_classes_.p, d_basis_tiles_e_.p, n_basis_tiles_, basis_pad_, cheb_.n_pad, k, C, d_Lc_.p, d_L_.p, stream_);
        phase_end(kPhM2L2);
    }
    HIPCHK(hipGetLastError());
    (void)t;
    return BBFMM_OK;
}

int FmmTree::downward_tail(int k, const DownwardPlan *dp, const TargetSet *wx) {
    const HostTree &t = tree_;
    const int64_t C = t.n_cells();
    phase_begin();
    if (t.adaptive && wx) {
        launch_wx_sym(kernel_, cheb_, wx->n_wx_jobs, wx->wx_tb.p, wx->wx_te.p, wx->wx_range.p, wx->n_wxl_jobs, wx->wxl_tb.p, wx->wxl_te.p,
                      wx->wxl_range.p, d_w_idx_.p, d_centers_.p,
                      d_lengths_.p, src_ptr_, d_w_sorted_.p, t.n_points, k, d_M_.p, d_L_.p, C * cheb_.n_pad, wx->out.p,
                      static_cast<int64_t>(wx->m), wx->sym_off, static_cast<int>(wx->m), stream_);
    } else if (t.adaptive) {
        if (dp)
            launch_p2l(kernel_, cheb_, dp->n_x_jobs, dp->d_x_cells.p, dp->d_x_ptr.p, dp->d_x_runs.p, d_centers_.p,
                       d_lengths_.p, src_ptr_, d_w_sorted_.p, t.n_points, k, C, d_L_.p, stream_);
        else
            launch_p2l(kernel_, cheb_, static_cast<int>(x_cells_.size()), d_x_cells_.p, d_x_job_run_ptr_.p,
                       d_x_runs_.p, d_centers_.p, d_lengths_.p, src_ptr_, d_w_sorted_.p, t.n_points, k, C, d_L_.p,
                       stream_);
    }
    phase_end(kPhP2L);
    phase_begin();
    for (int level = 2; level <= t.depth; ++level) {
// ... 700 lines not shown
```

ferreus_rbf_rs_amd/csrc/fmm_tree.hpp:

```cpp
#pragma once
#include <hip/hip_runtime.h>

#include <cstdint>
#include <string>
#include <memory>
#include <vector>

#include "device.hpp"
#include "targets.hpp"
#include "ferreus_bbfmm_hip.h"
#include "kernels.hpp"
#include "operators.hpp"
#include "parallel.hpp"
#include "tree.hpp"
#include "tree_device.hpp"

namespace bbfmm {

enum Phase {
    kPhGather = 0, kPhP2M, kPhM2M, kPhM2L1, kPhM2L2, kPhP2L, kPhL2L, kPhP2P, kPhM2P, kPhL2P, kPhScatter,
    kNumPhases
};
static_assert(kNumPhases == BBFMM_N_PHASES, "phase table");

template <class T> struct DevBuf {
    T *p = nullptr;
    size_t n = 0;
    bool borrowed = false;
};

struct HostM2lClass {
    int level = 0, octant = 0;
    int n_rows = 0, r_pad16 = 16, n_t = 0, k_pad = 16;
    std::vector<double> vt_all, u_all;
    std::vector<int> src_tv, tgt_tv, tgt_off;
    std::vector<int32_t> row_tpos, row_off, row_dst, blk_t0, cells;
    std::vector<int32_t, DefaultInitAllocator<int32_t>> cslot;
    std::vector<int32_t> src_row0, src_row1;
    std::vector<int32_t> row_tpos2, row_off2, row_dst2;
    std::vector<int32_t> src_pair;
    int kp = 0;
    std::vector<int32_t> tgt_pair;
    std::vector<int64_t> cbase;
};

struct M2lBatch {
    int level_lo = 0, level_hi = 0;
    int groups = 1, group = 0;
    int64_t len = 0;
    int32_t t1_first = 0, t1_count = 0;
    int32_t t2_first = 0, t2_count = 0;
};

struct TargetSet {
    int64_t m = 0;
    DevBuf<double> xyz[3];
    const double *xyz_ptr[3] = {nullptr, nullptr, nullptr};
    DevBuf<int32_t> perm;
    DevBuf<int32_t> job_cell, tgt_begin, tgt_end;
    int n_jobs = 0;
    DevBuf<int32_t> w_tgt_begin, w_tgt_end;
    DevBuf<int64_t> w_begin, w_end;
    int n_w_jobs = 0;
    DevBuf<double> out, grad;
    bool sym = false;
    int32_t sym_off = 0;
    int n_sym_jobs = 0;
    DevBuf<int32_t> sym_tb, sym_te;
    DevBuf<int64_t> sym_ptr;
    DevBuf<int32_t> sym_runs;
    int n_syml_jobs = 0;
    DevBuf<int32_t> syml_tb, syml_te;
    DevBuf<int64_t> syml_ptr;
    int n_symw_jobs = 0;
    DevBuf<int32_t> symw_tb, symw_te;
    DevBuf<int64_t> symw_ptr;
    int n_wx_jobs = 0;
    DevBuf<int32_t> wx_tb, wx_te;
    DevBuf<int64_t> wx_range;
    int n_wxl_jobs = 0;
    DevBuf<int32_t> wxl_tb, wxl_te;
    DevBuf<int64_t> wxl_range;
};

struct DownwardPlan {
    std::vector<uint8_t> active;
    std::vector<M2lTileDesc> tiles2_h;
    std::vector<M2lTileDesc> tiles1_h;
    std::vector<int32_t> batch_t1, batch_t2;
    int64_t n_tiles1_blocks = 0;
    std::vector<int32_t> tile_idx_h;
    std::vector<uint16_t> qlist_h;
    int n_x_jobs = 0;
// ... 52 lines not shown
    bool is_identity_subset(const int64_t *idx, int64_t n_idx) const;
    int fast_matrix_vector_product(const double *w, int64_t rows, int64_t basis_size, const int64_t *target_indices,
                                   int64_t n_target_indices, const double *poly, int64_t ldp, double nugget,
                                   double *result);
    int matvec_device(const double *d_w, int64_t ldw, int k, double *d_out, int64_t ldo, bool sync);
    int64_t partition_coarse_count() const;
    int matvec_partition_upward(const double *d_w, int64_t ldw, int k, double *d_coarse, hipStream_t comm_stream, bool near_field = true);
    int partition_subset_finish(const double *d_coarse, const int64_t *idx, int64_t n_idx, double *h_out, hipStream_t comm_stream);
    int matvec_partition_finish(const double *d_coarse, double *d_out, int64_t ldo, bool sync, hipStream_t comm_stream);
    int matvec_partition_finish_sorted(const double *d_coarse, double *d_seg, int64_t ld, hipStream_t comm_stream);
    int partition_scatter(const double *d_all, int first_part, int n_parts, int64_t m_max, int k, double *d_out, int64_t ldo);
    int matvec_partition_finish_host(const double *d_coarse, double *h_seg, int64_t ld, hipStream_t comm_stream);
    const std::vector<int64_t> &partition_bounds() const { return part_bounds_; }
    int register_subset(const int64_t *idx, int64_t n_idx, int *id_out);
    int matvec_subset_device(int id, const double *d_w, double *d_y, bool sync);
    int set_partition(int rank, int world);

    const HostTree &tree() const { return tree_; }
    const Operators &ops() const { return ops_; }
    const PodDoubles &source_points() const { return pts_; }
    int order() const { return order_; }
    const char *last_error() const { return err_.c_str(); }
    hipStream_t stream() const { return stream_; }
    bool host_only() const { return host_only_; }
    void bind_device() const {
        if (device_ >= 0) (void)hipSetDevice(device_);
    }
    int device() const { return device_; }
    bool tree_built_on_device() const { return tree_built_on_device_; }
    bool last_evaluate_at_sources() const { return last_eval_at_sources_; }
    int last_evaluate_path() const { return last_eval_at_sources_ ? 1 : (last_eval_rows_of_sources_ ? 2 : 0); }
    bool targets_are_rows_of_sources(const double *x, int64_t m, int64_t ldx, std::vector<int64_t> *rows);
    bool targets_are_sources(const double *x, int64_t m, int64_t ldx) const;
    void stats(bbfmm_tree_stats *out) const;
    void set_profiling(bool on) { profiling_ = on; }
    const double *phase_ms() { collect_phase_times(); return phase_ms_; }
    const int64_t *phase_count() { collect_phase_times(); return phase_count_; }
    void reset_phase_ms() {
        collect_phase_times();
        for (double &v : phase_ms_) v = 0.0;
        for (int64_t &v : phase_count_) v = 0;
    }
    const std::vector<int64_t> &partition_rows() const { return part_rows_; }
    bool partitioned() const { return part_world_ > 1; }
    int partition_rank() const { return part_rank_; }
    const std::vector<HostM2lClass> &m2l_host() const { return m2l_host_; }
    void m2l_variant_stats(int64_t *n_variants, int64_t *n_cells) const {
        *n_variants = static_cast<int64_t>(m2l_variants_.size());
        *n_cells = 0;
        for (const HostM2lClass &v : m2l_variants_) *n_cells += static_cast<int64_t>(v.cells.size());
    }
    void debug_m2l_pairs(std::vector<int32_t> *out) const;
    bool m2l_pairs() const { return m2l_pairs_; }
    void debug_m2l_pairs_stage2(std::vector<int32_t> *out) const;
    bool m2l_pairs_stage2() const { return m2l_pairs2_; }
    int debug_m2l_s2_last_ksplit() const { return m2l_s2_last_ksplit_; }
    int debug_apply_m2l_tables_host(const double *M, double *L) const;
    int debug_get_coefficients(char which, int k, double *out);
    int debug_partition_upward_counts(int64_t *counts_out, uint8_t *reads_out, int64_t *info_out) const;

  private:
    int fail(int code, const std::string &msg);
    int hip_fail(hipError_t e, const char *what);
    int upload();
    int build_m2l_tables();
    void fill_m2l_operator_arrays(const HostM2lClass &hc, std::vector<double> *vt_all,
                                  std::vector<double> *u_all) const;
    void fill_m2l_operator_arrays(const HostM2lClass &hc, double *vt_all, double *u_all) const;
    int ensure_rhs_capacity(int k);
    int upward(int k, const DownwardPlan *dp = nullptr);
    int downward(int k, const DownwardPlan *dp = nullptr, const TargetSet *wx = nullptr);
    int downward_m2l(int k, const DownwardPlan *dp);
    int downward_tail(int k, const DownwardPlan *dp, const TargetSet *wx);
    int leaf_pass(const TargetSet &ts, int k, bool with_grads);
    int leaf_pass_near(const TargetSet &ts, int k, bool with_grads, hipStream_t st, int parts, bool wx_done = false);
    int leaf_pass_far(const TargetSet &ts, int k, bool with_grads);
    int build_target_set(const double *x, int64_t m, int64_t ldx, TargetSet *ts, int64_t *bad_point_index,
                         std::vector<int32_t> *leaves_out = nullptr);
    int build_target_set_device(const double *x, int64_t m, int64_t ldx, TargetSet *ts, int64_t *bad_point_index,
                                std::vector<int32_t> *leaves_out, const double *const *d_x = nullptr);
    int ensure_leaf_lookup();
    int build_target_set_host(const double *x, int64_t m, int64_t ldx, TargetSet *ts, int64_t *bad_point_index,
                              std::vector<int32_t> *leaves_out);
    int build_source_target_set();
    int build_sym_runs(TargetSet *ts, const std::vector<int32_t> &job_cells, int64_t pb, int64_t pe, const std::vector<uint8_t> *part_active = nullptr);
    void free_target_set(TargetSet *ts);
    hipError_t columns_to_host(double *dst, int64_t ld, const double *d_src, int64_t m, int ncols);
    int upload_weights(const double *w, int64_t rows, int k, int64_t ldw);
    void phase_begin();
    void phase_end(int ph);
    void collect_phase_times();
    hipEvent_t get_event();

    std::string err_;
    bool host_only_ = false;
    bool deterministic_ = false;
    bool tree_built_on_device_ = false;
    DevTreePoints dev_points_;
    int order_ = 0, d_ = 0;
    KernelSpec kernel_{};
    bbfmm_params params_{};
    PodDoubles pts_;
    HostTree tree_;
    Operators ops_;
    int nrhs_ = 0;
    bool have_locals_ = false;
    bool locals_requested_ = false;
    Csr u_runs_;
    Csr x_runs_;
    std::vector<int32_t> src_leaves_;
    std::vector<std::vector<int32_t>> m2m_parents_;
    std::vector<std::vector<int32_t>> level_cells_;
    std::vector<int32_t> x_cells_;
    std::vector<HostM2lClass> m2l_host_;
    std::vector<HostM2lClass> m2l_variants_;
    std::vector<M2lTileDesc> m2l_tiles1_h_;
    std::vector<int32_t> m2l_tile_idx1_h_;
    std::vector<M2lClass> m2l_classes_h_;
    std::vector<M2lTileDesc> m2l_tiles_h_;
    std::vector<uint16_t> m2l_qlist_h_;
    std::vector<M2lBatch> m2l_batches_;
    std::vector<int32_t> m2l_batch_of_class_;
    std::vector<std::vector<int32_t>> m2l_group_ops_;
    std::vector<int32_t> m2l_zero_h_;
    std::vector<int64_t> m2l_zero_ptr_;
    int64_t cbuf_batch_len_ = 0;
    int64_t cbuf_total_len_ = 0;
    int64_t m2l_budget_bytes_ = int64_t(16384) << 20;
    int m2l_rhs_chunk_ = 1;
    double m2l_flops_k1_ = 0;
    int n_cu_ = 256;
    int device_ = -1;
    std::vector<M2lTileDesc> m2l_tiles2_h_;
    int m2l_slot_t_ = 1;
    int m2l_max_blocks_ = 1;
    int m2l_s1_block_ = kM2lS1Block;
    bool m2l_pairs_ = false;
    int m2l_ne_ = 0, m2l_no_ = 0;
    int m2l_ne16_ = 0, m2l_npar_ = 0;
    std::vector<int32_t> m2l_partner_;
    int m2l_rho(int m) const {
        const int p1 = ops_.n / ops_.p;
        return m + (ops_.p - 1 - 2 * (m / p1)) * p1;
    }
    DevBuf<double> d_Mp_;
    bool m2l_pairs2_ = false;
    M2lS2PairsPlan m2l_s2_plan_{1, 1, 1, 1};
    DevBuf<double> d_Lp_;
    int m2l_s2_last_ksplit_ = 0;
    int part_rank_ = 0, part_world_ = 1;
    std::vector<int64_t> part_rows_, part_bounds_;
    int partition_finish_core(const double *d_coarse, hipStream_t comm_stream, int *k_out);
    bool part_empty_ = false;
    DownwardPlan part_plan_;
    std::vector<std::unique_ptr<SubsetPlan>> subset_plans_;
    uint64_t subset_clock_ = 0;
    int build_downward_plan(const std::vector<int32_t> &target_leaves, DownwardPlan *dp, bool restrict_upward = false,
                            int64_t own_b = 0, int64_t own_e = 0);
    int part_pending_k_ = 0;
    bool multipoles_partial_ = false;
    void free_downward_plan(DownwardPlan *dp);
    int subset_plan(const int64_t *idx, int64_t n_idx, SubsetPlan **out);
    uint64_t subset_key(const int64_t *idx, int64_t n_idx) const;
    bool subset_plan_cached(const int64_t *idx, int64_t n_idx, uint64_t key) const;
    uint64_t last_subset_miss_ = 0;
    int fill_subset_plan(const int64_t *idx, int64_t n_idx, SubsetPlan *sp);
    std::vector<std::unique_ptr<SubsetPlan>> registered_plans_;

    hipStream_t stream_ = nullptr;
    hipEvent_t ev_pack_ = nullptr, ev_comm_ = nullptr;
    struct PendingPhase {
        int phase;
        hipEvent_t e0, e1;
    };
    std::vector<PendingPhase> pending_;
    std::vector<hipEvent_t> event_pool_;
    hipEvent_t pending_begin_ = nullptr;
    bool profiling_ = false;
    double phase_ms_[kNumPhases] = {0};
    int64_t phase_count_[kNumPhases] = {0};
    std::vector<void *> owned_;
    template <class T> int dalloc(DevBuf<T> *b, size_t n, bool zero = false);
    template <class T> int dupload(DevBuf<T> *b, const std::vector<T> &v);
    template <class T> int talloc(DevBuf<T> *b, size_t n, bool zero = false);
    template <class T> int tupload(DevBuf<T> *b, const std::vector<T> &v);
    void arena_begin();
    int arena_end();
    template <class T> void dfree(DevBuf<T> *b);

    ChebRef cheb_{};
    DevBuf<DevCheb> d_cheb_;
    DevBuf<double> d_src_[3];
    const double *src_ptr_[3] = {nullptr, nullptr, nullptr};
// ... 75 lines not shown
```

ferreus_rbf_rs_amd/fmm_tree.py:

```python
from __future__ import annotations

import ctypes
import enum
from typing import Optional

import numpy as np

from . import _lib as L


class KernelType(enum.IntEnum):
    LinearRbf = 0
    ThinPlateSplineRbf = 1
    CubicRbf = 2
    Spheroidal3Rbf = 3
    Spheroidal5Rbf = 4
    Spheroidal7Rbf = 5
    Spheroidal9Rbf = 6
    Laplacian = 7
    OneOverR2 = 8
    OneOverR4 = 9
    GaussianExt = 100
    MultiquadricExt = 101

# ... 420 lines not shown

    def permutation_tables(self):
        n = self.stats().n_nodes
        nperm = ctypes.c_int32(0)
        self._raise(self._lib.bbfmm_get_permutation_tables(self._h, ctypes.byref(nperm), None, None,
                                                           None, None))
        nvec = 7 ** self.dim
        perm = np.zeros((nperm.value, n), dtype=np.int32)
        inv = np.zeros((nperm.value, n), dtype=np.int32)
        pl = np.zeros(nvec, dtype=np.int32)
        rl = np.zeros(nvec, dtype=np.int32)
        self._raise(self._lib.bbfmm_get_permutation_tables(
            self._h, ctypes.byref(nperm), perm.ctypes.data, inv.ctypes.data, pl.ctypes.data,
            rl.ctypes.data))
        return perm, inv, pl, rl

    def points_to_leaves(self, x):
        x = self._targets(x)
        m = x.shape[0]
        cells = np.zeros(max(m, 1), dtype=np.int32)
        bad = ctypes.c_int64(-1)
        rc = self._lib.bbfmm_points_to_leaves(self._h, x.ctypes.data, m, max(m, 1),
                                              cells.ctypes.data, ctypes.byref(bad))
        self._raise(rc, bad)
        return cells[:m]

    def debug_dense_m2m(self, child_index: int):
        n = self.stats().n_nodes
        out = np.zeros((n, n), order="F")
        self._raise(self._lib.bbfmm_debug_dense_m2m(self._h, child_index, out.ctypes.data))
        return out

    def debug_m2l_variants(self):
        nv, nc = ctypes.c_int64(), ctypes.c_int64()
        self._raise(self._lib.bbfmm_debug_m2l_variants(self._h, ctypes.byref(nv), ctypes.byref(nc)))
        return nv.value, nc.value

    def debug_m2l_pairs(self, stage=1):
        fn = self._lib.bbfmm_debug_m2l_pairs if stage == 1 else self._lib.bbfmm_debug_m2l_pairs_stage2
        n, on = ctypes.c_int64(), ctypes.c_int32()
        self._raise(fn(self._h, None, 0, ctypes.byref(n), ctypes.byref(on)))
        buf = np.zeros(max(n.value, 1), dtype=np.int32)
        self._raise(fn(self._h, buf.ctypes.data, n.value, ctypes.byref(n), ctypes.byref(on)))
        d, ops, i = self.dim, [], 0
        while i < n.value:
            level, octant, kind, ne = (int(v) for v in buf[i:i + 4])
            ent = buf[i + 4:i + 4 + ne * (d + 1)].reshape(ne, d + 1)
            ops.append({"level": level, "octant": octant, "kind": kind,
                        "pairs": [tuple(int(x) for x in e[1:]) for e in ent if e[0] == 1],
                        "singles": [tuple(int(x) for x in e[1:]) for e in ent if e[0] == 0]})
            i += 4 + ne * (d + 1)
        return bool(on.value), ops

    def debug_m2l_s2_last_ksplit(self) -> int:
        ks = ctypes.c_int32()
        self._raise(self._lib.bbfmm_debug_m2l_s2_last_ksplit(self._h, ctypes.byref(ks)))
        return ks.value

    def debug_get_coefficients(self, which: str, k: int) -> np.ndarray:
        s = self.stats()
        out = np.zeros((k, s.n_cells, s.n_nodes))
        self._raise(self._lib.bbfmm_debug_get_coefficients(self._h, which.encode()[0:1], k,
                                                           out.ctypes.data))
        return out

    def debug_apply_m2l_tables_host(self, M: np.ndarray) -> np.ndarray:
        M = np.ascontiguousarray(M, dtype=np.float64)
        Lc = np.zeros_like(M)
        self._raise(self._lib.bbfmm_debug_apply_m2l_tables_host(self._h, M.ctypes.data,
                                                                Lc.ctypes.data))
        return Lc


def fp64_valu_selftest():
    tf, mhz = ctypes.c_double(0), ctypes.c_double(0)
    if L.load().bbfmm_fp64_valu_selftest(ctypes.byref(tf), ctypes.byref(mhz)) != L.OK:
        raise RuntimeError("the FP64 VALU microbenchmark needs a HIP device")
    return tf.value, mhz.value


def mfma_f64_selftest():
    tf = ctypes.c_double(0)
    errs = ctypes.c_int32(-1)
    info = (ctypes.c_double * 6)()
    rc = L.load().bbfmm_mfma_f64_selftest(ctypes.byref(tf), ctypes.byref(errs), info)
    if rc != L.OK:
        raise RuntimeError("MFMA self-test needs a HIP device")
    mfma_f64_selftest.info = dict(zip(["cycles_per_mfma_lone_wave", "clock_mhz_lone_wave",
                                       "cycles_per_mfma_per_simd_busy", "clock_mhz_busy",
                                       "tflops_1wave_per_simd", "tflops_2waves_per_simd"], list(info)))
    return tf.value, errs.value


def debug_kernel_values(where: int, kernel_id: int, base_range: float, total_sill: float, r2):
    x = np.ascontiguousarray(r2, dtype=np.float64).ravel()
    v, vg, f = np.empty_like(x), np.empty_like(x), np.empty_like(x)
    rc = L.load().bbfmm_debug_kernel_values(where, kernel_id, float(base_range), float(total_sill), x.ctypes.data, x.size,
                                            v.ctypes.data, vg.ctypes.data, f.ctypes.data)
    if rc != L.OK:
        raise RuntimeError(f"bbfmm_debug_kernel_values failed with status {rc}")
    return v, vg, f


DEBUG_MATH = {"sqrt": 0, "sqrt_rsqrt": 1, "rcp": 2, "log": 3}


# ... 9 lines not shown
```

include/ferreus_bbfmm_hip.h:

```cpp
#ifndef FERREUS_BBFMM_HIP_H
#define FERREUS_BBFMM_HIP_H

#include <stdint.h>

#ifdef __cplusplus
extern "C" {
#endif

typedef enum {
    BBFMM_OK = 0,
    BBFMM_POINT_OUTSIDE_TREE = 1,
    BBFMM_KERNEL_NO_GRADIENTS = 2,
    BBFMM_BAD_ARGUMENT = 3,
    BBFMM_DEVICE_ERROR = 4,
    BBFMM_UNSUPPORTED = 5
} bbfmm_status;

typedef enum {
    BBFMM_KERNEL_LINEAR_RBF = 0,
    BBFMM_KERNEL_THIN_PLATE_SPLINE_RBF = 1,
    BBFMM_KERNEL_CUBIC_RBF = 2,
    BBFMM_KERNEL_SPHEROIDAL3_RBF = 3,
    BBFMM_KERNEL_SPHEROIDAL5_RBF = 4,
    BBFMM_KERNEL_SPHEROIDAL7_RBF = 5,
// ... 177 lines not shown

int bbfmm_debug_host_copy_rates(int64_t n, double *out4);

typedef struct {
    int32_t d, order, n_nodes, depth;
    int64_t n_points, n_cells, n_leaves;
    int64_t n_u, n_v, n_w, n_x;
    int64_t p2p_pairs;
    int64_t p2p_tile_bytes_k1;
    double m2l_flops_k1;
    double center[3];
    double radius;
    int64_t wx_pairs;
    int64_t wx_tile_bytes_k1;
    int32_t m2l_basis_rank;
    int32_t m2l_basis_len;
    int32_t m2l_batches;
    int32_t m2l_rhs_per_pass;
    int64_t m2l_slots_bytes_per_rhs;
    int64_t m2l_intermediate_bytes;
} bbfmm_tree_stats;

int bbfmm_get_tree_stats(const bbfmm_handle *h, bbfmm_tree_stats *out);
int bbfmm_tree_built_on_device(const bbfmm_handle *h);

int bbfmm_get_cells(const bbfmm_handle *h, uint64_t *keys, uint8_t *is_leaf);
int bbfmm_get_leaf_sources(const bbfmm_handle *h, int64_t *ptr, int64_t *idx);
int bbfmm_get_list(const bbfmm_handle *h, char which, int64_t *ptr, int32_t *idx,
                   int64_t *n_entries);
int bbfmm_get_m2l_ranks(const bbfmm_handle *h, int32_t *ranks, int32_t *n_ref_out);
int bbfmm_get_m2l_operator(const bbfmm_handle *h, int32_t level, int32_t ref, double *out);
int bbfmm_get_m2l_factors(const bbfmm_handle *h, int32_t level, int32_t ref, double *u, double *vt);
int bbfmm_get_permutation_tables(const bbfmm_handle *h, int32_t *n_perm, int32_t *perm,
                                 int32_t *invperm, int32_t *perm_lookup, int32_t *ref_lookup);
int bbfmm_points_to_leaves(const bbfmm_handle *h, const double *x, int64_t m, int64_t ldx,
                           int32_t *cell_out, int64_t *bad_point_index);

#define BBFMM_N_PHASES 11
int bbfmm_set_profiling(bbfmm_handle *h, int32_t enable);
int bbfmm_get_phase_ms(bbfmm_handle *h, double *ms_out, int64_t *count_out);
int bbfmm_reset_phase_ms(bbfmm_handle *h);

int bbfmm_mfma_f64_selftest(double *tflops, int32_t *layout_errors, double *info6);
int bbfmm_fp64_valu_selftest(double *tflops, double *clock_mhz);

int bbfmm_debug_kernel_values(int32_t where, int32_t kernel_id, double base_range, double total_sill, const double *r2,
                              int64_t n, double *value_out, double *value_g_out, double *factor_out);
int bbfmm_debug_math(int32_t where, int32_t which, const double *x, int64_t n, double *out, double *out2);

int bbfmm_debug_dense_m2m(const bbfmm_handle *h, int32_t child_index, double *out);
int bbfmm_debug_apply_m2l_tables_host(const bbfmm_handle *h, const double *M, double *L);
int bbfmm_debug_m2l_variants(const bbfmm_handle *h, int64_t *n_variants, int64_t *n_cells);
int bbfmm_debug_m2l_pairs(const bbfmm_handle *h, int32_t *out, int64_t cap, int64_t *n_out, int32_t *pairs_on);
int bbfmm_debug_m2l_pairs_stage2(const bbfmm_handle *h, int32_t *out, int64_t cap, int64_t *n_out, int32_t *pairs_on);
int bbfmm_debug_m2l_s2_last_ksplit(const bbfmm_handle *h, int32_t *ksplit);

uint64_t bbfmm_debug_morton_encode(int32_t d, const uint64_t *anchor, uint64_t level);
void bbfmm_debug_morton_decode(int32_t d, uint64_t key, uint64_t *anchor_out, uint64_t *level_out);
int32_t bbfmm_debug_morton_neighbours(int32_t d, uint64_t key, uint64_t *keys_out);
int32_t bbfmm_debug_direction_vectors(int32_t d, int32_t *out);
int bbfmm_debug_reference_vectors(const bbfmm_handle *h, int32_t *out, int32_t *n_ref_out);

int bbfmm_debug_get_coefficients(bbfmm_handle *h, char which, int32_t k, double *out);


typedef int (*bbfmm_apply_fn)(void *user, const double *x, double *y, int64_t n);
typedef void (*bbfmm_iteration_fn)(void *user, int64_t iter, double residual, double progress);

enum { BBFMM_ACCURACY_ABSOLUTE = 0, BBFMM_ACCURACY_RELATIVE = 1 };

void bbfmm_givens_rotation(double f, double g, double *c, double *s, double *r);

int bbfmm_fgmres(int64_t n, bbfmm_apply_fn a, void *a_user, const double *b, bbfmm_apply_fn m, void *m_user,
                 const double *x0, int32_t max_outer_iterations, int32_t max_inner_iterations,
                 int32_t tolerance_type, double tolerance, bbfmm_iteration_fn callback, void *cb_user,
                 double *x, int64_t *iterations, double *final_residual);

int bbfmm_schwarz_ddm_solver(int64_t n, bbfmm_apply_fn matvec, void *a_user, const double *rhs,
                             bbfmm_apply_fn m, void *m_user, int32_t max_iterations, int32_t tolerance_type,
                             double tolerance, bbfmm_iteration_fn callback, void *cb_user, double *x,
                             int64_t *iterations, double *final_residual);

typedef struct bbfmm_rbf_system {
    bbfmm_handle *tree;
    int64_t basis_size;
    const double *monomial_matrix;
    int64_t ld_monomial;
    double nugget;
} bbfmm_rbf_system;
int bbfmm_rbf_system_apply(void *user, const double *x, double *y, int64_t n);

typedef struct bbfmm_ddm bbfmm_ddm;
typedef struct bbfmm_ddm_params {
    int64_t leaf_threshold;
    double overlap_quota;
    double coarse_ratio;
    int64_t coarse_threshold;
} bbfmm_ddm_params;
void bbfmm_ddm_params_defaults(bbfmm_ddm_params *out);
void bbfmm_ddm_params_for_points(int64_t n, bbfmm_ddm_params *out);
int bbfmm_ddm_build(const double *points, int64_t n, int32_t d, int64_t ld, const bbfmm_ddm_params *params,
                    bbfmm_ddm **out);
void bbfmm_ddm_destroy(bbfmm_ddm *t);
int32_t bbfmm_ddm_num_levels(const bbfmm_ddm *t);
int64_t bbfmm_ddm_level_size(const bbfmm_ddm *t, int32_t level);
int bbfmm_ddm_level_points(const bbfmm_ddm *t, int32_t level, int64_t *out);
// ... 51 lines not shown
```

Measured before the change: 30.19 matvecs/s.

## Extend M2L stage-1 parity folding to pair M2L operators along the y axis too

Adds a second reflection axis (y) to the M2L parity-pairing scheme. Interaction vectors related by a y-mirror now share one stage-1 GEMM via even/odd splits of the multipole coefficients. A new parity2 kernel builds four parity blocks (ee, eo, oe, oo), and a matching assembly kernel produces the combined VT basis. Stage 1 swaps eo/oe column segments for y-paired blocks. The aim is to shrink the stage-1 M2L GEMM work, at the cost of more complex setup and the risk of padding overhead or a wrong column mapping.

Measured after the change: 31.94 matvecs/s, median of 6. +5.8%, better.

```diff
diff --git a/ferreus_rbf_rs_amd/_lib.py b/ferreus_rbf_rs_amd/_lib.py
--- a/ferreus_rbf_rs_amd/_lib.py
+++ b/ferreus_rbf_rs_amd/_lib.py
@@ -132,6 +132,7 @@
     "bbfmm_debug_apply_m2l_tables_host": (ctypes.c_int, [c_p, c_p, c_p]),
     "bbfmm_debug_m2l_variants": (ctypes.c_int, [c_p, c_p, c_p]),
     "bbfmm_debug_m2l_pairs": (ctypes.c_int, [c_p, c_p, c_i64, c_p, c_p]),
+    "bbfmm_debug_m2l_pairs_axes": (ctypes.c_int, [c_p, c_p, c_i64, c_p]),
     "bbfmm_debug_m2l_pairs_stage2": (ctypes.c_int, [c_p, c_p, c_i64, c_p, c_p]),
     "bbfmm_debug_m2l_s2_last_ksplit": (ctypes.c_int, [c_p, c_p]),
     "bbfmm_debug_get_coefficients": (ctypes.c_int, [c_p, ctypes.c_char, c_i32, c_p]),
diff --git a/ferreus_rbf_rs_amd/csrc/capi.cpp b/ferreus_rbf_rs_amd/csrc/capi.cpp
--- a/ferreus_rbf_rs_amd/csrc/capi.cpp
+++ b/ferreus_rbf_rs_amd/csrc/capi.cpp
@@ -1297,6 +1297,15 @@
     return BBFMM_OK;
 }
 
+int bbfmm_debug_m2l_pairs_axes(const bbfmm_handle *h, int32_t *out, int64_t cap, int64_t *n_out) {
+    if (!h || !n_out) return BBFMM_BAD_ARGUMENT;
+    std::vector<int32_t> v;
+    h->tree.debug_m2l_pairs_axes(&v);
+    *n_out = static_cast<int64_t>(v.size());
+    if (out) std::copy(v.begin(), v.begin() + std::min<int64_t>(cap, *n_out), out);
+    return BBFMM_OK;
+}
+
 int bbfmm_debug_m2l_pairs_stage2(const bbfmm_handle *h, int32_t *out, int64_t cap, int64_t *n_out, int32_t *pairs_on) {
     if (!h || !n_out) return BBFMM_BAD_ARGUMENT;
     std::vector<int32_t> v;
diff --git a/ferreus_rbf_rs_amd/csrc/device.hpp b/ferreus_rbf_rs_amd/csrc/device.hpp
--- a/ferreus_rbf_rs_amd/csrc/device.hpp
+++ b/ferreus_rbf_rs_amd/csrc/device.hpp
@@ -31,6 +31,7 @@
     const int32_t *row_dst;
     const int32_t *row_dst2;
     const int32_t *blk_t0;
+    int32_t yb0;
     int32_t n_rows;
     int32_t r_pad16;
     int32_t n_t;
@@ -82,9 +83,15 @@
 
 void launch_m2l_stage1(const M2lClass *classes, const M2lTileDesc *tiles, const int32_t *tile_idx, int n_tiles,
                        int n_pad, int max_slot_t, int K, int64_t C, const double *M, double *cbuf,
-                       int64_t cbuf_len, hipStream_t s, bool own_blocks = false, int max_blocks = 8, int ne16 = 0);
+                       int64_t cbuf_len, hipStream_t s, bool own_blocks = false, int max_blocks = 8, int ne16 = 0, int s_ee = 0,
+                       int s_eo = 0);
 void launch_m2l_parity(const double *M, int n_pad, double *Mp, int n_par, int ne16, int n_e, int n_o, int p, int64_t rows,
                        hipStream_t s);
+struct M2lParityOffsets {
+    int32_t v[4];
+};
+void launch_m2l_parity2(const double *M, int n_pad, double *Mp, int n_par, M2lParityOffsets off, int p, int p2, int64_t rows,
+                        hipStream_t s);
 void launch_m2l_stage2(const M2lClass *classes, const M2lTileDesc *tiles, const int32_t *tile_idx, int n_tiles,
                        int n_pad, int K, int64_t C, const double *cbuf, int64_t cbuf_len,
                        const uint16_t *qlist, double *L, hipStream_t s, bool allow_ksplit = true);
@@ -117,6 +124,8 @@
     int32_t n_src, n_tgt, r_pad16, k_pad, max_rank;
     int32_t n_e, n_o, ne16, n_par, p;
     int32_t u_npar, u_ne16, u_rows, u_ne, u_no;
+    int32_t s1_axes;
+    M2lParityOffsets s1_off;
 };
 void launch_m2l_assemble(const M2lAssembleClass &c, int n, int n_pad, bool compressed, const double *ops,
                          const int32_t *invperm, double *vt_all, double *u_all, hipStream_t s);
diff --git a/ferreus_rbf_rs_amd/csrc/device_m2l.hip b/ferreus_rbf_rs_amd/csrc/device_m2l.hip
--- a/ferreus_rbf_rs_amd/csrc/device_m2l.hip
+++ b/ferreus_rbf_rs_amd/csrc/device_m2l.hip
@@ -71,7 +71,8 @@
     const int q_lo = STAGE == 2 ? tile.q_count * zk / ksplit : 0;
     const int nq = STAGE == 1 ? n_pad / 16 : STAGE == 2 ? tile.q_count * (zk + 1) / ksplit - q_lo : (int)(in_len / 16);
     const uint16_t *ql = qlist + tile.q_first + q_lo;
-    const int nq_e = PAIRS ? (int)(in_len / 16) : 0;
+    const int nq_e = PAIRS ? (int)(in_len & 0xffffffff) / 16 : 0;
+    const int s_ee = PAIRS ? (int)(in_len >> 32) & 0xffff : 0, s_eo = PAIRS ? (int)(in_len >> 48) : 0;
     if (zb0 >= zb1) return;
     const int g16 = g16_0 + (STAGE >= 2 ? zc * NG16 : 0);
     const double *opbase = (STAGE == 1 ? cls.vt_all : cls.u_all) + 16 * g16;
@@ -112,7 +113,13 @@
     const int64_t qstride = (int64_t)16 * ld;
     auto stage = [&](int sidx, int buf) {
         const int zb = zb0 + sidx / nq, qi = sidx - (sidx / nq) * nq;
-        const int q = STAGE == 2 ? (int)ql[qi] : qi;
+        int q = STAGE == 2 ? (int)ql[qi] : qi;
+        if constexpr (PAIRS) {
+            if (zb >= cls.yb0) {
+                if (qi >= s_ee && qi < s_ee + s_eo) q = qi + s_eo;
+                else if (qi >= s_ee + s_eo && qi < s_ee + 2 * s_eo) q = qi - s_eo;
+            }
+        }
 #pragma unroll
         for (int i = 0; i < NCH; ++i)
             if (wave + 8 * i < OP_CHUNKS)
@@ -403,7 +410,7 @@
 
 void launch_m2l_stage1(const M2lClass *classes, const M2lTileDesc *tiles, const int32_t *tile_idx, int n_tiles,
                        int n_pad, int max_slot_t, int K, int64_t C, const double *M, double *cbuf, int64_t cbuf_len,
-                       hipStream_t s, bool own_blocks, int max_blocks, int ne16) {
+                       hipStream_t s, bool own_blocks, int max_blocks, int ne16, int s_ee, int s_eo) {
     if (n_tiles == 0) return;
     int slot_t = 16;
     while (slot_t < max_slot_t) slot_t *= 2;
@@ -421,7 +428,8 @@
     }
     const int n_colblocks = own_blocks ? 1 : zsplit;
     if (ne16 > 0) {
-        m2l_gemm_launch<kM2lS1BlockPairs / 16, 1, 1, true>(classes, tiles, n_tiles, n_pad, 0, n_colblocks, K, C, M, ne16, cbuf, cbuf_len,
+        const int64_t packed = static_cast<int64_t>(ne16) | (static_cast<int64_t>(s_ee & 0xffff) << 32) | (static_cast<int64_t>(s_eo & 0x7fff) << 48);
+        m2l_gemm_launch<kM2lS1BlockPairs / 16, 1, 1, true>(classes, tiles, n_tiles, n_pad, 0, n_colblocks, K, C, M, packed, cbuf, cbuf_len,
                                                       nullptr, slot_t, tile_idx, s);
         return;
     }
@@ -717,6 +725,35 @@
     const int p1 = n_e / ((p + 1) / 2);
     hipLaunchKernelGGL(m2l_parity_kernel, dim3(static_cast<unsigned>((rows + 3) / 4)), dim3(256), 0, s, M, n_pad, Mp, n_par, ne16, n_e,
                        n_o, p, p1, rows);
+}
+
+__global__ __launch_bounds__(256) void m2l_parity2_kernel(const double *__restrict__ M, int n_pad, double *__restrict__ Mp, int n_par,
+                                                          M2lParityOffsets off, int p, int p2, int64_t rows) {
+    const int64_t row = static_cast<int64_t>(blockIdx.x) * 4 + (threadIdx.x >> 6);
+    if (row >= rows) return;
+    const double *src = M + row * n_pad;
+    double *dst = Mp + row * n_par;
+    const int h = (p + 1) / 2, f = p / 2;
+    for (int e = threadIdx.x & 63; e < h * h * p2; e += 64) {
+        const int i0 = e / (h * p2), i1 = (e - i0 * h * p2) / p2, r = e - (i0 * h + i1) * p2;
+        const int m = (i0 * p + i1) * p2 + r;
+        const int dx = (p - 1 - 2 * i0) * p * p2, dy = (p - 1 - 2 * i1) * p2;
+        const bool cx = i0 >= f, cy = i1 >= f;
+        const double v = src[m], vx = src[m + dx], vy = src[m + dy], vxy = src[m + dx + dy];
+        const double e0 = cx ? v : v + vx, e1 = cx ? vy : vy + vxy, o0 = v - vx, o1 = vy - vxy;
+        const int je = (i0 * h + i1) * p2 + r, jo = (i0 * f + i1) * p2 + r;
+        dst[off.v[0] + je] = cy ? e0 : e0 + e1;
+        if (!cy) dst[off.v[1] + jo] = e0 - e1;
+        if (!cx) dst[off.v[2] + je] = cy ? o0 : o0 + o1;
+        if (!cx && !cy) dst[off.v[3] + jo] = o0 - o1;
+    }
+}
+
+void launch_m2l_parity2(const double *M, int n_pad, double *Mp, int n_par, M2lParityOffsets off, int p, int p2, int64_t rows,
+                        hipStream_t s) {
+    if (rows <= 0) return;
+    hipLaunchKernelGGL(m2l_parity2_kernel, dim3(static_cast<unsigned>((rows + 3) / 4)), dim3(256), 0, s, M, n_pad, Mp, n_par, off, p, p2,
+                       rows);
 }
 
 __global__ __launch_bounds__(256) void m2l_zero_segments_kernel(const int32_t *__restrict__ segs, int64_t n_segs,
@@ -832,6 +869,38 @@
     }
 }
 
+__global__ __launch_bounds__(256) void assemble_vt_parity2_kernel(M2lAssembleClass c, int n, const double *__restrict__ ops,
+                                                                  const int32_t *__restrict__ invperm, double *__restrict__ vt_all) {
+    const int p = c.p, p2 = n / (p * p), h = (p + 1) / 2, f = p / 2, n_ee = h * h * p2;
+    const int64_t t = static_cast<int64_t>(blockIdx.x) * 256 + threadIdx.x;
+    if (t >= static_cast<int64_t>(c.n_src) * n_ee) return;
+    const int pos = static_cast<int>(t / n_ee), e = static_cast<int>(t % n_ee);
+    const M2lAssembleTv tv = c.src[pos];
+    const int i0 = e / (h * p2), i1 = (e - i0 * h * p2) / p2, r = e - (i0 * h + i1) * p2;
+    const int m = (i0 * p + i1) * p2 + r;
+    const int dx = (p - 1 - 2 * i0) * p * p2, dy = (p - 1 - 2 * i1) * p2;
+    const bool cx = i0 >= f, cy = i1 >= f;
+    const int32_t *inv = invperm + static_cast<int64_t>(tv.perm) * n;
+    const double *s0 = ops + tv.vt_off + static_cast<int64_t>(inv[m]) * tv.rank;
+    const double *sx = ops + tv.vt_off + static_cast<int64_t>(inv[m + dx]) * tv.rank;
+    const double *sy = ops + tv.vt_off + static_cast<int64_t>(inv[m + dy]) * tv.rank;
+    const double *sxy = ops + tv.vt_off + static_cast<int64_t>(inv[m + dx + dy]) * tv.rank;
+    const int je = (i0 * h + i1) * p2 + r, jo = (i0 * f + i1) * p2 + r;
+    double *dee = vt_all + static_cast<int64_t>(c.s1_off.v[0] + je) * c.r_pad16 + tv.row;
+    double *deo = vt_all + static_cast<int64_t>(c.s1_off.v[1] + jo) * c.r_pad16 + tv.row;
+    double *doe = vt_all + static_cast<int64_t>(c.s1_off.v[2] + je) * c.r_pad16 + tv.row;
+    double *doo = vt_all + static_cast<int64_t>(c.s1_off.v[3] + jo) * c.r_pad16 + tv.row;
+    const double wx = cx ? 1.0 : 0.5, wy = cy ? 1.0 : 0.5;
+    for (int kk = 0; kk < tv.rank; ++kk) {
+        const double v = s0[kk], vx = sx[kk], vy = sy[kk], vxy = sxy[kk];
+        const double e0 = cx ? v : v + vx, e1 = cx ? vy : vy + vxy, o0 = v - vx, o1 = vy - vxy;
+        dee[kk] = wx * wy * (cy ? e0 : e0 + e1);
+        if (!cy) deo[kk] = wx * wy * (e0 - e1);
+        if (!cx) doe[kk] = wx * wy * (cy ? o0 : o0 + o1);
+        if (!cx && !cy) doo[kk] = wx * wy * (o0 - o1);
+    }
+}
+
 __global__ __launch_bounds__(256) void assemble_u_kernel(M2lAssembleClass c, int n, int n_pad, const double *__restrict__ ops,
                                                          const int32_t *__restrict__ invperm, double *__restrict__ u_all) {
     const int pos = blockIdx.y;
@@ -867,7 +936,11 @@
                          const int32_t *invperm, double *vt_all, double *u_all, hipStream_t s) {
     (void)hipMemsetAsync(vt_all, 0, static_cast<size_t>(c.n_e > 0 ? c.n_par : n_pad) * c.r_pad16 * sizeof(double), s);
     (void)hipMemsetAsync(u_all, 0, (c.u_npar > 0 ? static_cast<size_t>(c.u_rows) * c.u_npar : static_cast<size_t>(c.k_pad) * n_pad) * sizeof(double), s);
-    if (c.n_src > 0 && c.n_e > 0)
+    if (c.n_src > 0 && c.n_e > 0 && c.s1_axes == 2) {
+        const int h = (c.p + 1) / 2, n_ee = h * h * (n / (c.p * c.p));
+        hipLaunchKernelGGL(assemble_vt_parity2_kernel, dim3(static_cast<unsigned>((static_cast<int64_t>(c.n_src) * n_ee + 255) / 256)), dim3(256),
+                           0, s, c, n, ops, invperm, vt_all);
+    } else if (c.n_src > 0 && c.n_e > 0)
         hipLaunchKernelGGL(assemble_vt_parity_kernel, dim3(static_cast<unsigned>((static_cast<int64_t>(c.n_src) * c.n_e + 255) / 256)), dim3(256),
                            0, s, c, n, ops, invperm, vt_all);
     else if (c.n_src > 0)
diff --git a/ferreus_rbf_rs_amd/csrc/fmm_m2l_tables.cpp b/ferreus_rbf_rs_amd/csrc/fmm_m2l_tables.cpp
--- a/ferreus_rbf_rs_amd/csrc/fmm_m2l_tables.cpp
+++ b/ferreus_rbf_rs_amd/csrc/fmm_m2l_tables.cpp
@@ -33,7 +33,26 @@
         const M2lOperator &op = lops[ops_.ref_lookup[tv]];
         row_src.push_back(RowSrc{&op, &ops_.invperm[static_cast<size_t>(ops_.perm_lookup[tv]) * n], hc.src_row0[pos]});
     }
-    if (m2l_pairs_) {
+    if (m2l_pairs_ && m2l_axes_ == 2) {
+        parallel_for(m2l_npar_, 8, [&](int64_t k) {
+            const int32_t *nd = &m2l_par_node_[static_cast<size_t>(4 * k)];
+            const int8_t *sg = &m2l_par_sign_[static_cast<size_t>(4 * k)];
+            int cnt = 0;
+            for (int g = 0; g < 4; ++g) cnt += nd[g] >= 0;
+            if (cnt == 0) return;
+            const double w = 1.0 / cnt;
+            double *dst = vt_all + static_cast<size_t>(k) * hc.r_pad16;
+            for (const RowSrc &rs : row_src) {
+                const int r = rs.op->rank;
+                for (int kk = 0; kk < r; ++kk) {
+                    double v = 0.0;
+                    for (int g = 0; g < 4; ++g)
+                        if (nd[g] >= 0) v += sg[g] * rs.op->vt[static_cast<size_t>(rs.inv[nd[g]]) * r + kk];
+                    dst[rs.first_row + kk] = w * v;
+                }
+            }
+        });
+    } else if (m2l_pairs_) {
         parallel_for(m2l_ne_, 8, [&](int64_t j) {
             const bool centre = j >= m2l_no_;
             const int rj = m2l_rho(static_cast<int>(j));
@@ -162,6 +181,22 @@
             for (int m = 0; m < n && ok; ++m) ok = ir[m] == it[m2l_rho(m)];
             if (ok) m2l_partner_[static_cast<size_t>(tv)] = rt;
         }
+        m2l_partner_y_.assign(static_cast<size_t>(nvec), -1);
+        for (int tv = 0; tv < nvec && m2l_pairs_; ++tv) {
+            if (comp(tv, 1) == 0) continue;
+            int rt = -1;
+            for (int u = 0; u < nvec && rt < 0; ++u) {
+                bool same = comp(u, 1) == -comp(tv, 1);
+                for (int a = 0; a < d; ++a) same = same && (a == 1 || comp(u, a) == comp(tv, a));
+                if (same) rt = u;
+            }
+            if (rt < 0 || ops_.ref_lookup[rt] != ops_.ref_lookup[tv]) continue;
+            const int32_t *it = &ops_.invperm[static_cast<size_t>(ops_.perm_lookup[tv]) * n];
+            const int32_t *ir = &ops_.invperm[static_cast<size_t>(ops_.perm_lookup[rt]) * n];
+            bool ok = true;
+            for (int m = 0; m < n && ok; ++m) ok = ir[m] == it[m2l_rho_y(m)];
+            if (ok) m2l_partner_y_[static_cast<size_t>(tv)] = rt;
+        }
     }
     auto far = [&](int tv) {
         int mx = 0;
@@ -210,6 +245,145 @@
     for (int o = 0; o < ncls; ++o) {
         if (m2l_pairs_) pairs_first(&src_list[o], &tpos_src[o]);
         if (m2l_pairs2_) pairs_first(&tgt_list[o], &tpos_tgt[o]);
+    }
+    auto order_axes = [&](std::vector<int> *list, std::vector<int> *carry) {
+        const size_t nl = list->size();
+        std::vector<int> where(static_cast<size_t>(nvec), -1);
+        for (size_t i = 0; i < nl; ++i) where[static_cast<size_t>((*list)[i])] = static_cast<int>(i);
+        std::vector<uint8_t> used(nl, 0);
+        std::vector<size_t> order, ypairs;
+        for (int pass = 0; pass < 2; ++pass) {
+            const std::vector<int32_t> &partner = pass == 0 ? m2l_partner_ : m2l_partner_y_;
+            for (size_t i = 0; i < nl; ++i) {
+                if (used[i]) continue;
+                const int tv = (*list)[i], rt = partner[static_cast<size_t>(tv)];
+                const int j = rt >= 0 ? where[static_cast<size_t>(rt)] : -1;
+                if (j < 0 || used[static_cast<size_t>(j)] || partner[static_cast<size_t>(rt)] != tv) continue;
+                const bool lead = comp(tv, pass) > 0;
+                std::vector<size_t> &dst = pass == 0 ? order : ypairs;
+                dst.push_back(lead ? i : static_cast<size_t>(j));
+                dst.push_back(lead ? static_cast<size_t>(j) : i);
+                used[i] = used[static_cast<size_t>(j)] = 1;
+            }
+        }
+        for (size_t i = 0; i < nl; ++i)
+            if (!used[i]) order.push_back(i);
+        order.insert(order.end(), ypairs.begin(), ypairs.end());
+        std::vector<int> l2(nl), c2(nl);
+        for (size_t i = 0; i < nl; ++i) {
+            l2[i] = (*list)[order[i]];
+            if (carry) c2[i] = (*carry)[order[i]];
+        }
+        *list = l2;
+        if (carry) *carry = c2;
+    };
+    auto mark_pairs_at = [&](int level, int axes, const std::vector<int> &tvs, std::vector<int32_t> *src_pair, std::vector<int32_t> *row0,
+                             std::vector<int8_t> *kind, int *yb, int *pad) {
+        const auto &lops = ops_.m2l[level];
+        src_pair->assign(tvs.size(), -1);
+        std::vector<int8_t> kd(tvs.size(), 0);
+        for (size_t pos = 0; m2l_pairs_ && pos + 1 < tvs.size(); ++pos) {
+            const size_t a = static_cast<size_t>(tvs[pos]), b = static_cast<size_t>(tvs[pos + 1]);
+            const bool px = m2l_partner_[a] == tvs[pos + 1] && m2l_partner_[b] == tvs[pos];
+            const bool py = !px && axes == 2 && m2l_partner_y_[a] == tvs[pos + 1] && m2l_partner_y_[b] == tvs[pos];
+            if (px || py) {
+                (*src_pair)[pos] = static_cast<int32_t>(pos + 1);
+                (*src_pair)[pos + 1] = -2;
+                kd[pos] = kd[pos + 1] = px ? 1 : 2;
+                ++pos;
+            }
+        }
+        if (row0) row0->assign(tvs.size(), 0);
+        int rows = 0, blk = -1, blk_first = 0;
+        int last_x_blk = -1, y_blk = -1, pad_rows = 0;
+        for (size_t pos = 0; pos < tvs.size(); ++pos) {
+            if ((*src_pair)[pos] == -2) continue;
+            const int r = lops[ops_.ref_lookup[tvs[pos]]].rank;
+            if (r == 0) continue;
+            if (kd[pos] == 2 && y_blk < 0) {
+                if (rows / m2l_s1_block_ <= last_x_blk) {
+                    pad_rows = round_up(rows, m2l_s1_block_) - rows;
+                    rows += pad_rows;
+                }
+                y_blk = rows / m2l_s1_block_;
+            }
+            const int last = (*src_pair)[pos] >= 0 ? static_cast<int>(pos) + 1 : static_cast<int>(pos);
+            if (rows / m2l_s1_block_ == blk && last - blk_first + 1 > kM2lSlotWindow) rows = round_up(rows, m2l_s1_block_);
+            if (row0) (*row0)[pos] = rows;
+            const int b1 = (rows + r - 1) / m2l_s1_block_;
+            if (rows / m2l_s1_block_ != blk || b1 != blk) {
+                blk = b1;
+                blk_first = static_cast<int>(pos);
+            }
+            if (kd[pos] == 1) last_x_blk = b1;
+            rows = round_up(rows + r, 2);
+        }
+        if (kind) *kind = kd;
+        if (yb) *yb = y_blk;
+        if (pad) *pad = pad_rows;
+        return rows;
+    };
+    m2l_axes_ = 1;
+    m2l_s_ee_ = m2l_s_eo_ = 0;
+    m2l_s1_off_ = M2lParityOffsets{{0, m2l_ne16_, m2l_ne16_, m2l_npar_}};
+    m2l_work_[0] = m2l_work_[1] = 0;
+    m2l_par_node_.clear();
+    m2l_par_sign_.clear();
+    if (m2l_pairs_) {
+        const int p = ops_.p, p2 = n / (p * p), h = (p + 1) / 2, f = p / 2;
+        const int len[4] = {h * h * p2, h * f * p2, f * h * p2, f * f * p2};
+        M2lParityOffsets off2{{0, 0, 0, 0}};
+        for (int i = 1; i < 4; ++i) off2.v[i] = off2.v[i - 1] + round_up(len[i - 1], 16);
+        const int npar2 = off2.v[3] + round_up(len[3], 16);
+        std::vector<std::vector<int>> src_xy = src_list;
+        for (int o = 0; o < ncls; ++o) order_axes(&src_xy[o], nullptr);
+        for (int level = 2; level <= t.depth; ++level) {
+            std::vector<uint8_t> has(static_cast<size_t>(ncls), 0);
+            for (int64_t c = t.level_ptr[level]; c < t.level_ptr[level + 1]; ++c) has[t.octant[c]] = 1;
+            for (int o = 0; o < ncls; ++o) {
+                if (!has[static_cast<size_t>(o)]) continue;
+                std::vector<int32_t> marks;
+                const int rows1 = mark_pairs_at(level, 1, src_list[o], &marks, nullptr, nullptr, nullptr, nullptr);
+                const int rows2 = mark_pairs_at(level, 2, src_xy[o], &marks, nullptr, nullptr, nullptr, nullptr);
+                m2l_work_[0] += static_cast<int64_t>(round_up(std::max(rows1, 1), m2l_s1_block_) / m2l_s1_block_) * (m2l_npar_ / 16);
+                m2l_work_[1] += static_cast<int64_t>(round_up(std::max(rows2, 1), m2l_s1_block_) / m2l_s1_block_) * (npar2 / 16);
+            }
+        }
+        const char *e = std::getenv("BBFMM_M2L_S1_AXES");
+        const int want = e ? std::atoi(e) : 0;
+        if (want == 2 || (want != 1 && m2l_work_[1] < m2l_work_[0])) {
+            m2l_axes_ = 2;
+            m2l_s1_off_ = off2;
+            m2l_ne16_ = off2.v[2];
+            m2l_npar_ = npar2;
+            m2l_s_ee_ = off2.v[1] / 16;
+            m2l_s_eo_ = (off2.v[2] - off2.v[1]) / 16;
+            for (int o = 0; o < ncls; ++o) {
+                src_list[o] = src_xy[o];
+                for (size_t i = 0; i < src_list[o].size(); ++i) tpos_src[o][src_list[o][i]] = static_cast<int>(i);
+            }
+            m2l_par_node_.assign(static_cast<size_t>(npar2) * 4, -1);
+            m2l_par_sign_.assign(static_cast<size_t>(npar2) * 4, 0);
+            for (int i0 = 0; i0 < h; ++i0)
+                for (int i1 = 0; i1 < h; ++i1)
+                    for (int r = 0; r < p2; ++r) {
+                        const int m = (i0 * p + i1) * p2 + r;
+                        const bool cx = i0 >= f, cy = i1 >= f;
+                        const int nodes[4] = {m, m2l_rho(m), m2l_rho_y(m), m2l_rho_y(m2l_rho(m))};
+                        const int je = (i0 * h + i1) * p2 + r, jo = (i0 * f + i1) * p2 + r;
+                        for (int part = 0; part < 4; ++part) {
+                            const bool ox = part >= 2, oy = part & 1;
+                            if ((ox && cx) || (oy && cy)) continue;
+                            const size_t k = static_cast<size_t>(off2.v[part] + (oy ? jo : je));
+                            for (int g = 0; g < 4; ++g) {
+                                const bool gx = g & 1, gy = g & 2;
+                                if ((gx && cx) || (gy && cy)) continue;
+                                m2l_par_node_[4 * k + g] = nodes[g];
+                                m2l_par_sign_[4 * k + g] = static_cast<int8_t>(((gx && ox) != (gy && oy)) ? -1 : 1);
+                            }
+                        }
+                    }
+        }
     }
     std::vector<std::vector<int32_t>> tgt_pair(ncls);
     for (int o = 0; o < ncls; ++o) {
@@ -324,38 +498,16 @@
         std::vector<int> k_pad, kp_cls;
         slot_layout(level, &off_tgt, &k_pad, &kp_cls);
         const size_t first_class = m2l_host_.size();
-        auto mark_pairs = [&](const std::vector<int> &tvs, std::vector<int32_t> *src_pair, std::vector<int32_t> *row0 = nullptr) {
-            src_pair->assign(tvs.size(), -1);
-            for (size_t pos = 0; m2l_pairs_ && pos + 1 < tvs.size(); ++pos)
-                if (m2l_partner_[static_cast<size_t>(tvs[pos])] == tvs[pos + 1] && m2l_partner_[static_cast<size_t>(tvs[pos + 1])] == tvs[pos]) {
-                    (*src_pair)[pos] = static_cast<int32_t>(pos + 1);
-                    (*src_pair)[pos + 1] = -2;
-                    ++pos;
-                }
-            if (row0) row0->assign(tvs.size(), 0);
-            int rows = 0, blk = -1, blk_first = 0;
-            for (size_t pos = 0; pos < tvs.size(); ++pos) {
-                if ((*src_pair)[pos] == -2) continue;
-                const int r = rank_of(tvs[pos]);
-                if (r == 0) continue;
-                const int last = (*src_pair)[pos] >= 0 ? static_cast<int>(pos) + 1 : static_cast<int>(pos);
-                if (rows / m2l_s1_block_ == blk && last - blk_first + 1 > kM2lSlotWindow) rows = round_up(rows, m2l_s1_block_);
-                if (row0) (*row0)[pos] = rows;
-                const int b1 = (rows + r - 1) / m2l_s1_block_;
-                if (rows / m2l_s1_block_ != blk || b1 != blk) {
-                    blk = b1;
-                    blk_first = static_cast<int>(pos);
-                }
-                rows = round_up(rows + r, 2);
-            }
-            return rows;
+        auto mark_pairs = [&](const std::vector<int> &tvs, std::vector<int32_t> *src_pair) {
+            return mark_pairs_at(level, m2l_axes_, tvs, src_pair, nullptr, nullptr, nullptr, nullptr);
         };
         auto stage1_rows = [&](int o, const std::vector<int> &tvs, HostM2lClass *hcp) {
             HostM2lClass &hc = *hcp;
             hc.n_t = static_cast<int>(tvs.size());
             std::vector<int32_t> first_row;
-            hc.n_rows = mark_pairs(tvs, &hc.src_pair, &first_row);
+            hc.n_rows = mark_pairs_at(level, m2l_axes_, tvs, &hc.src_pair, &first_row, &hc.src_kind, &hc.yb0, &hc.pad_cols);
             hc.r_pad16 = round_up(std::max(hc.n_rows, 1), m2l_s1_block_);
+            if (hc.yb0 < 0) hc.yb0 = hc.r_pad16 / m2l_s1_block_;
             hc.row_tpos.assign(hc.r_pad16, -1);
             hc.row_off.assign(hc.r_pad16, 0);
             hc.row_tpos2.assign(hc.r_pad16, -1);
@@ -582,6 +734,7 @@
                     }
                 }
                 if (tvs.empty()) continue;
+                if (m2l_axes_ == 2) order_axes(&tvs, &keep);
                 HostM2lClass v;
                 v.level = level;
                 v.octant = o;
@@ -648,9 +801,13 @@
                 while (j < nc && same_pattern(i, j)) ++j;
                 size_t full = 0;
                 if (variants_on && j - i >= static_cast<size_t>(variant_min_tiles) * kM2lTile) {
-                    std::vector<int> tvs;
+                    std::vector<int> tvs, keep;
                     for (int ps = 0; ps < nt; ++ps)
-                        if (hc.cslot[i * nt + ps] >= 0) tvs.push_back(hc.src_tv[ps]);
+                        if (hc.cslot[i * nt + ps] >= 0) {
+                            tvs.push_back(hc.src_tv[ps]);
+                            keep.push_back(ps);
+                        }
+                    if (m2l_axes_ == 2) order_axes(&tvs, &keep);
                     std::vector<int32_t> marks;
                     const int present_rows = mark_pairs(tvs, &marks);
                     auto n_pairs = [](const std::vector<int32_t> &m) { return std::count_if(m.begin(), m.end(), [](int32_t v) { return v >= 0; }); };
@@ -664,9 +821,6 @@
                         v.cells.assign(hc.cells.begin() + static_cast<std::ptrdiff_t>(i), hc.cells.begin() + static_cast<std::ptrdiff_t>(i + full));
                         v.cslot.resize(full * tvs.size());
                         size_t pv = 0;
-                        std::vector<int> keep;
-                        for (int ps = 0; ps < nt; ++ps)
-                            if (hc.cslot[i * nt + ps] >= 0) keep.push_back(ps);
                         for (size_t k = 0; k < full; ++k)
                             for (int ps : keep) v.cslot[pv++] = hc.cslot[(i + k) * nt + ps];
                         for (size_t f = 0; f < full; f += kM2lTile) {
@@ -1001,7 +1155,11 @@
         for (int64_t c = 0; c < tree_.n_cells(); ++c) {
             const double *Mv = M + static_cast<size_t>(c) * n;
             double *mp = &Mp[static_cast<size_t>(c) * m2l_npar_];
-            for (int j = 0; j < m2l_ne_; ++j) {
+            for (int k = 0; m2l_axes_ == 2 && k < m2l_npar_; ++k)
+                for (int g = 0; g < 4; ++g)
+                    if (m2l_par_node_[static_cast<size_t>(4 * k + g)] >= 0)
+                        mp[k] += m2l_par_sign_[static_cast<size_t>(4 * k + g)] * Mv[m2l_par_node_[static_cast<size_t>(4 * k + g)]];
+            for (int j = 0; m2l_axes_ == 1 && j < m2l_ne_; ++j) {
                 if (j < m2l_no_) {
                     mp[j] = Mv[j] + Mv[m2l_rho(j)];
                     mp[m2l_ne16_ + j] = Mv[j] - Mv[m2l_rho(j)];
@@ -1039,8 +1197,15 @@
                         if (slot < 0 && slot2 < 0) continue;
                         const double *mp = &Mp[static_cast<size_t>(hc.cells[pos]) * m2l_npar_];
                         double a = 0.0, bsum = 0.0;
-                        for (int j = 0; j < m2l_ne16_; ++j) a += hc.vt_all[static_cast<size_t>(j) * hc.r_pad16 + row] * mp[j];
-                        for (int j = m2l_ne16_; j < m2l_npar_; ++j) bsum += hc.vt_all[static_cast<size_t>(j) * hc.r_pad16 + row] * mp[j];
+                        if (row / m2l_s1_block_ >= hc.yb0) {
+                            for (int j = 0; j < m2l_npar_; ++j) {
+                                const bool y_odd = (j >= m2l_s1_off_.v[1] && j < m2l_s1_off_.v[2]) || j >= m2l_s1_off_.v[3];
+                                (y_odd ? bsum : a) += hc.vt_all[static_cast<size_t>(j) * hc.r_pad16 + row] * mp[j];
+                            }
+                        } else {
+                            for (int j = 0; j < m2l_ne16_; ++j) a += hc.vt_all[static_cast<size_t>(j) * hc.r_pad16 + row] * mp[j];
+                            for (int j = m2l_ne16_; j < m2l_npar_; ++j) bsum += hc.vt_all[static_cast<size_t>(j) * hc.r_pad16 + row] * mp[j];
+                        }
                         if (slot >= 0) cbuf[static_cast<size_t>(slot) * 2 + hc.row_off[row]] = a + bsum;
                         if (slot2 >= 0) cbuf[static_cast<size_t>(slot2) * 2 + hc.row_off2[row]] = a - bsum;
                         continue;
@@ -1111,8 +1276,42 @@
         out->push_back(0);
         int32_t n_entries = 0;
         for (size_t pos = 0; pos < h.src_tv.size(); ++pos) {
+            const bool x_pair = h.src_pair[pos] >= 0 && h.src_kind[pos] == 1;
+            if (h.src_pair[pos] == -2 && h.src_kind[pos] == 1) continue;
+            out->push_back(x_pair ? 1 : 0);
+            for (int a = 0; a < d; ++a) out->push_back(ops_.all_vecs[static_cast<size_t>(h.src_tv[pos]) * d + a]);
+            ++n_entries;
+        }
+        (*out)[n_at] = n_entries;
+    }
+}
+
+void FmmTree::debug_m2l_pairs_axes(std::vector<int32_t> *out) const {
+    out->clear();
+    const int d = d_;
+    out->push_back(m2l_pairs_ ? m2l_axes_ : 0);
+    out->push_back(static_cast<int32_t>(m2l_work_[0]));
+    out->push_back(static_cast<int32_t>(m2l_work_[1]));
+    for (size_t i = 0; i < m2l_host_.size() + m2l_variants_.size(); ++i) {
+        const HostM2lClass &h = i < m2l_host_.size() ? m2l_host_[i] : m2l_variants_[i - m2l_host_.size()];
+        if (h.cells.empty()) continue;
+        const int n_blk = h.r_pad16 / m2l_s1_block_;
+        out->push_back(h.level);
+        out->push_back(h.octant);
+        out->push_back(i < m2l_host_.size() ? 0 : 1);
+        out->push_back(h.pad_cols);
+        out->push_back(h.yb0);
+        out->push_back(n_blk);
+        const size_t n_at = out->size();
+        out->push_back(0);
+        for (int b = 0; b < n_blk; ++b) out->push_back(b >= h.yb0 ? 1 : 0);
+        int32_t n_entries = 0;
+        for (size_t pos = 0; pos < h.src_tv.size(); ++pos) {
             if (h.src_pair[pos] == -2) continue;
-            out->push_back(h.src_pair[pos] >= 0 ? 1 : 0);
+            out->push_back(h.src_pair[pos] >= 0 ? h.src_kind[pos] : 0);
+            const bool rows = h.src_row1[pos] > h.src_row0[pos];
+            out->push_back(rows ? h.src_row0[pos] / m2l_s1_block_ : -1);
+            out->push_back(rows ? (h.src_row1[pos] - 1) / m2l_s1_block_ : -1);
             for (int a = 0; a < d; ++a) out->push_back(ops_.all_vecs[static_cast<size_t>(h.src_tv[pos]) * d + a]);
             ++n_entries;
         }
diff --git a/ferreus_rbf_rs_amd/csrc/fmm_tree.cpp b/ferreus_rbf_rs_amd/csrc/fmm_tree.cpp
--- a/ferreus_rbf_rs_amd/csrc/fmm_tree.cpp
+++ b/ferreus_rbf_rs_amd/csrc/fmm_tree.cpp
@@ -476,6 +476,7 @@
         c.n_t = h.n_t;
         c.k_pad = h.k_pad;
         c.kp = h.kp;
+        c.yb0 = h.yb0;
         c.n_cells = static_cast<int32_t>(h.cells.size());
         if (h.cells.empty()) continue;
         DevBuf<double> vt, ua;
@@ -510,7 +511,8 @@
             const M2lAssembleClass ac{d_src.p, d_tgt.p, static_cast<int32_t>(src_tv.size()), static_cast<int32_t>(tgt_tv.size()),
                                       h.r_pad16, h.k_pad, max_rank,
                                       m2l_pairs_ ? m2l_ne_ : 0, m2l_no_, m2l_ne16_, m2l_npar_, ops_.p,
-                                      m2l_pairs2_ ? m2l_s2_plan_.n_par() : 0, m2l_s2_plan_.ne16(), h.k_pad - h.kp, m2l_ne_, m2l_no_};
+                                      m2l_pairs2_ ? m2l_s2_plan_.n_par() : 0, m2l_s2_plan_.ne16(), h.k_pad - h.kp, m2l_ne_, m2l_no_,
+                                      m2l_axes_, m2l_s1_off_};
             static const bool host_fill = std::getenv("BBFMM_M2L_ASSEMBLE_HOST") != nullptr;
             if (host_fill) {
                 std::vector<double> hv, hu;
@@ -873,7 +875,10 @@
     const int s1_len = m2l_pairs_ ? m2l_npar_ : m2l_len, s1_ne16 = m2l_pairs_ ? m2l_ne16_ : 0;
     if (m2l_pairs_ && !m2l_batches_.empty()) {
         phase_begin();
-        launch_m2l_parity(d_M_.p, cheb_.n_pad, d_Mp_.p, m2l_npar_, m2l_ne16_, m2l_ne_, m2l_no_, ops_.p, static_cast<int64_t>(k) * C, stream_);
+        if (m2l_axes_ == 2)
+            launch_m2l_parity2(d_M_.p, cheb_.n_pad, d_Mp_.p, m2l_npar_, m2l_s1_off_, ops_.p, ops_.n / (ops_.p * ops_.p), static_cast<int64_t>(k) * C, stream_);
+        else
+            launch_m2l_parity(d_M_.p, cheb_.n_pad, d_Mp_.p, m2l_npar_, m2l_ne16_, m2l_ne_, m2l_no_, ops_.p, static_cast<int64_t>(k) * C, stream_);
         phase_end(kPhM2L1);
     }
     double *l_out = shared_basis_ ? d_Lc_.p : s2_pairs ? d_Lp_.p : d_L_.p;
@@ -901,12 +906,12 @@
                                          cbuf_batch_len_, stream_);
             if (dp) {
                 launch_m2l_stage1(d_m2l_classes_.p, dp->d_tiles1.p + t1_first, dp->d_tile_idx.p, t1_count, s1_len, m2l_slot_t_, kb,
-                                  C, m_chunk, d_cbuf_.p, cbuf_batch_len_, stream_, false, m2l_max_blocks_, s1_ne16);
+                                  C, m_chunk, d_cbuf_.p, cbuf_batch_len_, stream_, false, m2l_max_blocks_, s1_ne16, m2l_s_ee_, m2l_s_eo_);
                 launch_m2l_stage1(d_m2l_classes_.p, dp->d_tiles1.p + dp->batch_t1[4 * b + 2], dp->d_tile_idx.p, dp->batch_t1[4 * b + 3],
-                                  s1_len, m2l_slot_t_, kb, C, m_chunk, d_cbuf_.p, cbuf_batch_len_, stream_, true, m2l_max_blocks_, s1_ne16);
+                                  s1_len, m2l_slot_t_, kb, C, m_chunk, d_cbuf_.p, cbuf_batch_len_, stream_, true, m2l_max_blocks_, s1_ne16, m2l_s_ee_, m2l_s_eo_);
             } else
                 launch_m2l_stage1(d_m2l_classes_.p, d_m2l_tiles1_.p + t1_first, d_tile_idx1_.p, t1_count, s1_len, m2l_slot_t_, kb, C,
-                                  m_chunk, d_cbuf_.p, cbuf_batch_len_, stream_, false, m2l_max_blocks_, s1_ne16);
+                                  m_chunk, d_cbuf_.p, cbuf_batch_len_, stream_, false, m2l_max_blocks_, s1_ne16, m2l_s_ee_, m2l_s_eo_);
             phase_end(kPhM2L1);
             phase_begin();
             if (s2_pairs) {
diff --git a/ferreus_rbf_rs_amd/csrc/fmm_tree.hpp b/ferreus_rbf_rs_amd/csrc/fmm_tree.hpp
--- a/ferreus_rbf_rs_amd/csrc/fmm_tree.hpp
+++ b/ferreus_rbf_rs_amd/csrc/fmm_tree.hpp
@@ -39,6 +39,9 @@
     std::vector<int32_t> src_row0, src_row1;
     std::vector<int32_t> row_tpos2, row_off2, row_dst2;
     std::vector<int32_t> src_pair;
+    std::vector<int8_t> src_kind;
+    int yb0 = 0;
+    int pad_cols = 0;
     int kp = 0;
     std::vector<int32_t> tgt_pair;
     std::vector<int64_t> cbase;
@@ -197,6 +200,7 @@
     }
     void debug_m2l_pairs(std::vector<int32_t> *out) const;
     bool m2l_pairs() const { return m2l_pairs_; }
+    void debug_m2l_pairs_axes(std::vector<int32_t> *out) const;
     void debug_m2l_pairs_stage2(std::vector<int32_t> *out) const;
     bool m2l_pairs_stage2() const { return m2l_pairs2_; }
     int debug_m2l_s2_last_ksplit() const { return m2l_s2_last_ksplit_; }
@@ -284,6 +288,17 @@
     int m2l_ne_ = 0, m2l_no_ = 0;
     int m2l_ne16_ = 0, m2l_npar_ = 0;
     std::vector<int32_t> m2l_partner_;
+    int m2l_axes_ = 1;
+    M2lParityOffsets m2l_s1_off_{{0, 0, 0, 0}};
+    int m2l_s_ee_ = 0, m2l_s_eo_ = 0;
+    int64_t m2l_work_[2] = {0, 0};
+    std::vector<int32_t> m2l_partner_y_;
+    std::vector<int32_t> m2l_par_node_;
+    std::vector<int8_t> m2l_par_sign_;
+    int m2l_rho_y(int m) const {
+        const int p2 = ops_.n / (ops_.p * ops_.p);
+        return m + (ops_.p - 1 - 2 * ((m / p2) % ops_.p)) * p2;
+    }
     int m2l_rho(int m) const {
         const int p1 = ops_.n / ops_.p;
         return m + (ops_.p - 1 - 2 * (m / p1)) * p1;
diff --git a/ferreus_rbf_rs_amd/fmm_tree.py b/ferreus_rbf_rs_amd/fmm_tree.py
--- a/ferreus_rbf_rs_amd/fmm_tree.py
+++ b/ferreus_rbf_rs_amd/fmm_tree.py
@@ -496,6 +496,24 @@
             i += 4 + ne * (d + 1)
         return bool(on.value), ops
 
+    def debug_m2l_pairs_axes(self):
+        fn = self._lib.bbfmm_debug_m2l_pairs_axes
+        n = ctypes.c_int64()
+        self._raise(fn(self._h, None, 0, ctypes.byref(n)))
+        buf = np.zeros(max(n.value, 1), dtype=np.int32)
+        self._raise(fn(self._h, buf.ctypes.data, n.value, ctypes.byref(n)))
+        info = {"axes": int(buf[0]), "work_x": int(buf[1]), "work_xy": int(buf[2])}
+        d, ops, i = self.dim, [], 3
+        while i < n.value:
+            level, octant, kind, pad_cols, yb0, n_blk, ne = (int(v) for v in buf[i:i + 7])
+            kinds = [int(v) for v in buf[i + 7:i + 7 + n_blk]]
+            ent = buf[i + 7 + n_blk:i + 7 + n_blk + ne * (d + 3)].reshape(ne, d + 3)
+            by_kind = [{tuple(int(x) for x in e[3:]): (int(e[1]), int(e[2])) for e in ent if e[0] == k} for k in range(3)]
+            ops.append({"level": level, "octant": octant, "kind": kind, "pad_cols": pad_cols, "yb0": yb0, "block_kinds": kinds,
+                        "singles": by_kind[0], "x_pairs": by_kind[1], "y_pairs": by_kind[2]})
+            i += 7 + n_blk + ne * (d + 3)
+        return info, ops
+
     def debug_m2l_s2_last_ksplit(self) -> int:
         ks = ctypes.c_int32()
         self._raise(self._lib.bbfmm_debug_m2l_s2_last_ksplit(self._h, ctypes.byref(ks)))
diff --git a/include/ferreus_bbfmm_hip.h b/include/ferreus_bbfmm_hip.h
--- a/include/ferreus_bbfmm_hip.h
+++ b/include/ferreus_bbfmm_hip.h
@@ -253,6 +253,7 @@
 int bbfmm_debug_apply_m2l_tables_host(const bbfmm_handle *h, const double *M, double *L);
 int bbfmm_debug_m2l_variants(const bbfmm_handle *h, int64_t *n_variants, int64_t *n_cells);
 int bbfmm_debug_m2l_pairs(const bbfmm_handle *h, int32_t *out, int64_t cap, int64_t *n_out, int32_t *pairs_on);
+int bbfmm_debug_m2l_pairs_axes(const bbfmm_handle *h, int32_t *out, int64_t cap, int64_t *n_out);
 int bbfmm_debug_m2l_pairs_stage2(const bbfmm_handle *h, int32_t *out, int64_t cap, int64_t *n_out, int32_t *pairs_on);
 int bbfmm_debug_m2l_s2_last_ksplit(const bbfmm_handle *h, int32_t *ksplit);
 
```
